# LiangZhaoPKUImperial/LinearSFM

Hardware: AMD Instinct MI355X
Metric: hierarchical linear map-joining solve wall-clock, NC3500-like stereo (all transforms + joins) (lower is better)
Workload: dtype f64

## Files before the change

include/lsfm.h:

```cpp
#ifndef LSFM_H
#define LSFM_H

#include <stddef.h>

#ifdef __cplusplus
extern "C" {
#endif

#define LSFM_OK 0
#define LSFM_ERR_ARG (-1)
#define LSFM_ERR_NO_DEVICE (-2)
#define LSFM_ERR_HIP (-3)
#define LSFM_ERR_OOM (-4)
#define LSFM_ERR_INTERNAL (-5)
#define LSFM_ERR_IO (-6)
#define LSFM_ERR_NOT_SPD (-7)
#define LSFM_NOT_CONVERGED 1

typedef struct lsfm_context lsfm_context;

typedef struct lsfm_map {
	int Ref, FRef, m, n, nU, nW;
	int ScaP, Fix, Sign, FScaP, FFix;
	int* stno;
// ... 75 lines not shown
int lsfm_gn_linearise_timed(lsfm_context* ctx, const lsfm_map* maps, int N, int type, const lsfm_map* x, const double* weight,
                            lsfm_map* out, double* obj, double* b, double* times, int* counts);
int lsfm_gn_linearise_features(lsfm_context* ctx, const lsfm_map* maps, int N, int type, const lsfm_map* x, const double* weight,
                               const double* fweight, lsfm_map* out, double* obj, double* b);
int lsfm_gn_linearise_features_timed(lsfm_context* ctx, const lsfm_map* maps, int N, int type, const lsfm_map* x, const double* weight,
                                     const double* fweight, lsfm_map* out, double* obj, double* b, double* times, int* counts);

int lsfm_map_covariance(lsfm_context* ctx, const lsfm_map* map, int mono, double* pose_cov, double* feat_cov, double* pair_cov, int cap_blocks, int* nnzb);
int lsfm_map_covariance_timed(lsfm_context* ctx, const lsfm_map* map, int mono, double* pose_cov, double* feat_cov, double* pair_cov, int cap_blocks, int* nnzb,
                              double* times);

int lsfm_map_covariance_columns(lsfm_context* ctx, const lsfm_map* map, int mono, const int* poses, int k, double* pose_cols, double* feat_cols,
                                double* joint, int* steps, double* last_corr);
int lsfm_map_covariance_columns_timed(lsfm_context* ctx, const lsfm_map* map, int mono, const int* poses, int k, double* pose_cols, double* feat_cols,
                                      double* joint, int* steps, double* last_corr, double* times);

int lsfm_map_covariance_feature_columns(lsfm_context* ctx, const lsfm_map* map, int mono, const int* feats, int k, double* pose_cols, double* feat_cols,
                                        double* joint, int* steps, double* last_corr);
int lsfm_map_feature_pair_gate(lsfm_context* ctx, const lsfm_map* map, int mono, const int* pairs, int K, double* d2, double* cov_diff, int* steps,
                               double* last_corr);
int lsfm_map_covariance_feature_columns_timed(lsfm_context* ctx, const lsfm_map* map, int mono, const int* feats, int k, double* pose_cols,
                                              double* feat_cols, double* joint, int* steps, double* last_corr, double* times);
int lsfm_map_feature_pair_gate_timed(lsfm_context* ctx, const lsfm_map* map, int mono, const int* pairs, int K, double* d2, double* cov_diff, int* steps,
                                     double* last_corr, double* times);

int lsfm_map_merge_features(lsfm_context* ctx, const lsfm_map* map, int mono, const int* pairs, int K, lsfm_map* out, double* d2, int* dof, int* rep,
                            int* steps, double* last_corr);
int lsfm_map_merge_features_timed(lsfm_context* ctx, const lsfm_map* map, int mono, const int* pairs, int K, lsfm_map* out, double* d2, int* dof,
                                  int* rep, int* steps, double* last_corr, double* times);
int lsfm_merge_structure(const lsfm_map* map, const int* pairs, int K, int* rep, int* photo, int* feature, int* FBlock, int* sptr, int* sidx, int cap_w,
                         int* info, char* why, int why_cap);

int lsfm_map_feature_pair_candidates(lsfm_context* ctx, const lsfm_map* map, const double* feat_cov, double radius, double tau, int* pairs, double* dist2,
                                     double* q, long long cap, long long* count);
int lsfm_map_feature_pair_candidates_timed(lsfm_context* ctx, const lsfm_map* map, const double* feat_cov, double radius, double tau, int* pairs,
                                           double* dist2, double* q, long long cap, long long* count, double* times, long long* info);

#define LSFM_JOINT_GATE_MAX 2048
int lsfm_map_feature_pair_joint_gate(lsfm_context* ctx, const lsfm_map* map, int mono, const int* pairs, int K, const int* order, double tau, int* status,
                                     double* delta, double* d2, double* joint_C, int* accepted, int* implied, double* D2, int* steps, double* last_corr);
int lsfm_map_feature_pair_joint_gate_timed(lsfm_context* ctx, const lsfm_map* map, int mono, const int* pairs, int K, const int* order, double tau,
                                           int* status, double* delta, double* d2, double* joint_C, int* accepted, int* implied, double* D2, int* steps,
                                           double* last_corr, double* times);
int lsfm_selftest_pair_select(lsfm_context* ctx, int K, const double* C, const double* d, const int* ends, const int* order, double tau, int* status,
                              double* delta, double* D2, int* accepted, int* implied);

int lsfm_map_marginalise(lsfm_context* ctx, const lsfm_map* map, const unsigned char* drop, lsfm_map* out);
int lsfm_map_marginalise_timed(lsfm_context* ctx, const lsfm_map* map, const unsigned char* drop, lsfm_map* out, double* times);

int lsfm_map_marginalise_poses(lsfm_context* ctx, const lsfm_map* map, int mono, const unsigned char* keep_pose, const unsigned char* drop_feat,
                               lsfm_map* out);
int lsfm_map_marginalise_poses_timed(lsfm_context* ctx, const lsfm_map* map, int mono, const unsigned char* keep_pose, const unsigned char* drop_feat,
                                     lsfm_map* out, double* times, int* info);
int lsfm_marg_pose_structure(const lsfm_map* map, int mono, const unsigned char* keep_pose, const unsigned char* drop_feat, unsigned char* drop,
                             int* comp, int* nptr, int* nidx, int cap_n, int* bd, int* Ui, int* Uj, int cap_u, int* info, char* why, int why_cap);

int lsfm_gn_structure(const lsfm_map* maps, int N, int type, const lsfm_map* x, int want_slots, int want_coalesce, int* info, int* map_hubs,
                      int* wdst, int* fptrJ, int* photoJ, int cap_wj, int* UiJ, int* UjJ, int cap_uj, int* photo, int* feature, int* FBlock,
                      int cap_w, int* Ui, int* Uj, int cap_u, int* slot_map, int* slot_a, int* slot_b, int* slot_count, int cap_s, char* why,
                      int why_cap);

int lsfm_inverse_v(lsfm_context* ctx, double* V, int m, int n);
int lsfm_solve_features(lsfm_context* ctx, const double* W, const double* IV, const double* ea, const double* eb, const double* dpa, double* dpb,
                        int m, int n, const int* mapCor, const int* photo);

int lsfm_schur_pattern(lsfm_context* ctx, const int* Ui, const int* Uj, const int* photo, const int* feature, int m, int n, int nU, int nW,
                       int* rowptr, int* colidx, int cap, int* nnzb);

int lsfm_symbolic_analyse(int m, const int* rowptr, const int* colidx, const int* origin, int reps, int* perm, int* colptr, int* rowidx,
                          int cap, int* info, double* avg_ms);

typedef struct lsfm_tree lsfm_tree;
int lsfm_tree_upload(lsfm_context* ctx, const lsfm_map* maps, int N, int mono, lsfm_tree** out);
int lsfm_tree_run(lsfm_context* ctx, lsfm_tree* tree, lsfm_stats* stats);
int lsfm_tree_set_final_reanchor(lsfm_tree* tree, int on);
int lsfm_tree_set_plans(lsfm_tree* tree, int on);
int lsfm_tree_download(lsfm_context* ctx, lsfm_tree* tree, lsfm_map* out);
int lsfm_tree_set_stop_level(lsfm_tree* tree, int levels);
int lsfm_tree_node_count(lsfm_context* ctx, lsfm_tree* tree);
int lsfm_tree_download_node(lsfm_context* ctx, lsfm_tree* tree, int k, lsfm_map* out);
int lsfm_tree_download_state(lsfm_context* ctx, lsfm_tree* tree, int* m, int* n, int* stno, double* stVal, size_t cap);
void lsfm_tree_free(lsfm_context* ctx, lsfm_tree* tree);
size_t lsfm_tree_export_size(lsfm_context* ctx, lsfm_tree* tree);
int lsfm_tree_export_dev(lsfm_context* ctx, lsfm_tree* tree, void* dst, size_t cap);
#define LSFM_PACK_HEADER_BYTES 256
size_t lsfm_packed_size(const void* host_header256);
int lsfm_tree_upload_dev(lsfm_context* ctx, const void* const* packed, int N, int mono, lsfm_tree** out);
int lsfm_tree_export_reduced_size(lsfm_context* ctx, lsfm_tree* tree, const int* keep_ids, int nkeep, size_t* bytes);
int lsfm_tree_export_reduced_dev(lsfm_context* ctx, lsfm_tree* tree, const int* keep_ids, int nkeep, void* dst, size_t cap);
int lsfm_tree_export_reduced_dev_timed(lsfm_context* ctx, lsfm_tree* tree, const int* keep_ids, int nkeep, void* dst, size_t cap, double* times);
int lsfm_tree_reload_dev(lsfm_context* ctx, lsfm_tree* tree, const void* const* packed, int N);

#define LSFM_DTYPE_F64 0
#define LSFM_DTYPE_I64 1
typedef int (*lsfm_allreduce_fn)(void* user, size_t offset_bytes, size_t count, int dtype, void* hip_stream);
int lsfm_tree_set_comm(lsfm_tree* tree, int rank, int world, lsfm_allreduce_fn fn, void* user, void* dev_buf, size_t dev_bytes);
int lsfm_tree_set_comm_blocks(lsfm_tree* tree, int block_maps);
int lsfm_tree_export_slice_sizes(lsfm_context* ctx, lsfm_tree* tree, int nslices, size_t* sizes);
int lsfm_tree_export_slice_dev(lsfm_context* ctx, lsfm_tree* tree, int nslices, int slice, void* dst, size_t cap);

int lsfm_divide_conquer(lsfm_context* ctx, const lsfm_map* maps, int N, int mono, lsfm_map* out, lsfm_stats* stats);

int lsfm_read_localmap(const char* path, int mono, lsfm_map* out);
int lsfm_read_localmaps(const char* dir, int first, int count, int mono, int threads, lsfm_map* out, int* failed);
int lsfm_write_localmap(const char* path, int mono, const lsfm_map* map);
int lsfm_write_mapset(const char* path, const lsfm_map* maps, int N, int mono);
int lsfm_mapset_info(const char* path, int* N, int* mono);
int lsfm_mapset_stamp(const char* path, unsigned long long* stamp, const unsigned long long* set_to);
int lsfm_read_mapset(const char* path, int mono, int first, int count, int threads, lsfm_map* out);
int lsfm_save_covariances(const char* pose_path, const char* feat_path, const int* stno, int m, int n, const double* pose_cov, const double* feat_cov);
int lsfm_read_covariances(const char* path, int k, int* ids, double* cov, int cap, int* count);
int lsfm_save_cov_columns(const char* path, const int* stno, int m, const int* poses, int k, const double* pose_cols);
int lsfm_read_cov_columns(const char* path, int* ids_q, int* ids_p, double* blocks, int cap, int* count);
int lsfm_save_pair_gate(const char* path, const int* ids, int K, const double* d2, const double* cov_diff);
int lsfm_read_pair_gate(const char* path, int* ids_f, int* ids_g, double* d2, double* cov_diff, int cap, int* count);
int lsfm_save_merge_report(const char* path, int K, int removed, int dof, double d2, const int* ids);
int lsfm_read_merge_report(const char* path, int* K, int* removed, int* dof, double* d2, int* ids, int cap);
int lsfm_save_joint_gate(const char* path, const int* ids, int K, const int* status, const double* d2, const double* delta, int accepted, int implied,
                         double D2);
int lsfm_read_joint_gate(const char* path, int* ids, int* status, double* d2, double* delta, int cap, int* head, double* D2);
int lsfm_save_pair_list(const char* path, const int* ids, long long K);
int lsfm_read_pair_list(const char* path, int* ids, long long cap, long long* count);
int lsfm_save_state(const char* path, const double* st, const int* stno, int n);
int lsfm_save_state_bin(const char* path, const double* st, const int* stno, int n);
int lsfm_save_poses(const char* pose_path, const char* feat_path, const int* stno, const double* st, int n);

int lsfm_spmv_bench(lsfm_context* ctx, int m, const int* rowptr, const int* colidx, const double* val,
                    const double* x, double* y, int reps, double* avg_ms, double* algorithmic_bytes);

int lsfm_wstream_bench(lsfm_context* ctx, long long nblocks, int mode, int reps, double* avg_ms);

int lsfm_selftest_prims(lsfm_context* ctx, int cases, unsigned seed);

int lsfm_selftest_vinv(lsfm_context* ctx, const double* V, const double* eb, int n, int skip, double* IV, double* LY);

#define LSFM_SELFTEST_CHOL_INFO 16
int lsfm_selftest_chol(lsfm_context* ctx, int m, const int* rowptr, const int* colidx, const double* val, const int* origin, const unsigned char* fixed,
                       const int* pose_seg, int nseg, const double* r, int nrhs, int mode, double* z, double* dot, int* perm, int* colptr, int* rowidx,
                       double* L, double* Dinv, double* dscale, int cap_blocks, int* info);

#define LSFM_SELFTEST_CC_SWEEPS_INFO 16
int lsfm_selftest_cc_sweeps(lsfm_context* ctx, int m, const int* rowptr, const int* colidx, const double* val, const int* origin,
                            const unsigned char* fixed, const double* B, int R, const double* X, double* x, double* fwd, int* perm, double* dscale,
                            double* y, int* info);

int lsfm_selftest_transform(lsfm_context* ctx, const lsfm_map* maps, int N, int mono, const int* tref, const int* tscap, const int* tfix,
                            int alias_passthrough, lsfm_map* out);

int lsfm_selftest_small(lsfm_context* ctx, int G, const int* pose_off, const int* feat_off, const int* u_off, const unsigned char* active,
                        const double* U, const int* Ui, const int* Uj, const double* W, const int* photo, const int* feature, int nW, const double* V,
                        const double* ea, const double* eb, const double* x0, const unsigned char* fixed, int strips, double* x_pose, double* x_feat,
                        int* status, double* max_rel);

#ifdef __cplusplus
}
#endif
#endif
```

linearsfm_amd/api.py:

```python
from __future__ import annotations

import ctypes as C
import os

import numpy as np

_HERE = os.path.dirname(os.path.abspath(__file__))
LIB_PATH = os.path.join(_HERE, "liblsfm_hip.so")
_LIB = None

LSFM_OK = 0
LSFM_NOT_CONVERGED = 1


class LsfmMap(C.Structure):
    _fields_ = [("Ref", C.c_int), ("FRef", C.c_int), ("m", C.c_int), ("n", C.c_int), ("nU", C.c_int), ("nW", C.c_int),
                ("ScaP", C.c_int), ("Fix", C.c_int), ("Sign", C.c_int), ("FScaP", C.c_int), ("FFix", C.c_int),
                ("stno", C.POINTER(C.c_int)), ("stVal", C.POINTER(C.c_double)),
                ("U", C.POINTER(C.c_double)), ("Ui", C.POINTER(C.c_int)), ("Uj", C.POINTER(C.c_int)),
                ("W", C.POINTER(C.c_double)), ("photo", C.POINTER(C.c_int)), ("feature", C.POINTER(C.c_int)),
                ("V", C.POINTER(C.c_double)), ("FBlock", C.POINTER(C.c_int)), ("pose_origin", C.POINTER(C.c_int))]


class LsfmStats(C.Structure):
    _fields_ = [("t_total_ms", C.c_double), ("t_transform_ms", C.c_double), ("t_join_ms", C.c_double),
                ("t_schur_ms", C.c_double), ("t_pcg_ms", C.c_double), ("t_backsub_ms", C.c_double),
                ("pcg_iterations", C.c_long), ("spmv_launches", C.c_long), ("spmv_ms", C.c_double),
                ("spmv_bytes", C.c_double), ("spmv_nnzb_upper_last", C.c_long), ("spmv_rows_last", C.c_long),
                ("max_rel_residual", C.c_double), ("levels", C.c_int), ("joins", C.c_int), ("transforms", C.c_int),
                ("not_converged", C.c_int), ("schur_launches", C.c_long), ("trf_launches", C.c_long),
                ("schur_ms", C.c_double), ("schur_bytes", C.c_double), ("trf_ms", C.c_double), ("trf_bytes", C.c_double),
                ("schur_flops", C.c_double), ("upload_ms", C.c_double), ("attempts", C.c_int),
                ("s_digest", C.c_ulonglong), ("factor_digest", C.c_ulonglong), ("dist_solves", C.c_int), ("dist_work_total", C.c_double), ("dist_work_shared", C.c_double), ("refactor_mismatch", C.c_int), ("s_rebuild_mismatch", C.c_int), ("small_levels", C.c_int), ("t_small_ms", C.c_double)]

    def as_dict(self):
        return {k: getattr(self, k) for k, _ in self._fields_}


class LsfmError(RuntimeError):
    pass


ALLREDUCE_FN = C.CFUNCTYPE(C.c_int, C.c_void_p, C.c_size_t, C.c_size_t, C.c_int, C.c_void_p)
LSFM_DTYPE_F64, LSFM_DTYPE_I64 = 0, 1
JOINT_GATE_MAX = 2048
JOINT_GATE_TAU = 11.344866730144373


def lib():
    global _LIB
    if _LIB is None:
        if not os.path.exists(LIB_PATH):
            raise LsfmError(f"{LIB_PATH} is missing: build it with `python -c 'import __graft_entry__ as g; g.build()'` "
                            "(hipcc --offload-arch=gfx950).  There is no CPU fallback.")
        L = C.CDLL(LIB_PATH)
        P = C.POINTER
        dp, ip, vp = P(C.c_double), P(C.c_int), C.c_void_p
        L.lsfm_context_create.argtypes = [C.c_int, C.c_size_t, P(vp)]
        L.lsfm_context_destroy.argtypes = [vp]
        L.lsfm_context_destroy.restype = None
        L.lsfm_set_pcg.argtypes = [vp, C.c_double, C.c_int]
        L.lsfm_set_precision.argtypes = [vp, C.c_int]
        L.lsfm_set_small_solve.argtypes = [vp, C.c_int]
        L.lsfm_set_spmv_variant.argtypes = [vp, C.c_int]
        L.lsfm_set_covcols_panel.argtypes = [vp, C.c_int]
        L.lsfm_last_error.argtypes = [vp]
        L.lsfm_last_error.restype = C.c_char_p
        L.lsfm_stream.argtypes = [vp]
        L.lsfm_stream.restype = vp
        L.lsfm_map_release.argtypes = [P(LsfmMap)]
        L.lsfm_map_release.restype = None
        L.lsfm_transform_stereo.argtypes = [vp, P(LsfmMap), C.c_int, P(LsfmMap)]
        L.lsfm_transform_mono.argtypes = [vp, P(LsfmMap), C.c_int, C.c_int, C.c_int, P(LsfmMap)]
        L.lsfm_join_stereo.argtypes = [vp, P(LsfmMap), P(LsfmMap), P(LsfmMap), dp, dp]
        L.lsfm_join_mono.argtypes = [vp, P(LsfmMap), P(LsfmMap), P(LsfmMap), dp, dp]
        L.lsfm_solve_stereo.argtypes = [vp, dp, dp, dp, dp, dp, dp, ip, ip, ip, ip, C.c_int, C.c_int, C.c_int, C.c_int, dp]
        L.lsfm_solve_mono.argtypes = [vp, dp, dp, dp, dp, dp, dp, ip, ip, ip, ip, C.c_int, C.c_int, C.c_int, C.c_int,
                                      C.c_int, C.c_int, C.c_int, C.c_int, C.c_int, dp]
        L.lsfm_tree_upload.argtypes = [vp, P(LsfmMap), C.c_int, C.c_int, P(vp)]
        L.lsfm_tree_run.argtypes = [vp, vp, P(LsfmStats)]
        L.lsfm_tree_set_final_reanchor.argtypes = [vp, C.c_int]
        L.lsfm_tree_set_plans.argtypes = [vp, C.c_int]
        L.lsfm_tree_export_size.argtypes = [vp, vp]
        L.lsfm_tree_export_size.restype = C.c_size_t
        L.lsfm_tree_export_dev.argtypes = [vp, vp, vp, C.c_size_t]
        L.lsfm_packed_size.argtypes = [vp]
        L.lsfm_packed_size.restype = C.c_size_t
        L.lsfm_tree_upload_dev.argtypes = [vp, P(vp), C.c_int, C.c_int, P(vp)]
        L.lsfm_tree_reload_dev.argtypes = [vp, vp, P(vp), C.c_int]
        L.lsfm_tree_set_comm.argtypes = [vp, C.c_int, C.c_int, ALLREDUCE_FN, vp, vp, C.c_size_t]
        L.lsfm_tree_set_comm_blocks.argtypes = [vp, C.c_int]
        L.lsfm_tree_export_slice_sizes.argtypes = [vp, vp, C.c_int, P(C.c_size_t)]
        L.lsfm_tree_export_slice_dev.argtypes = [vp, vp, C.c_int, C.c_int, vp, C.c_size_t]
        L.lsfm_tree_download.argtypes = [vp, vp, P(LsfmMap)]
        L.lsfm_tree_set_stop_level.argtypes = [vp, C.c_int]
        L.lsfm_tree_node_count.argtypes = [vp, vp]
        L.lsfm_tree_download_node.argtypes = [vp, vp, C.c_int, P(LsfmMap)]
        L.lsfm_tree_download_state.argtypes = [vp, vp, ip, ip, ip, dp, C.c_size_t]
        L.lsfm_tree_free.argtypes = [vp, vp]
        L.lsfm_tree_free.restype = None
        L.lsfm_divide_conquer.argtypes = [vp, P(LsfmMap), C.c_int, C.c_int, P(LsfmMap), P(LsfmStats)]
        L.lsfm_read_localmap.argtypes = [C.c_char_p, C.c_int, P(LsfmMap)]
        L.lsfm_write_localmap.argtypes = [C.c_char_p, C.c_int, P(LsfmMap)]
        L.lsfm_read_localmaps.argtypes = [C.c_char_p, C.c_int, C.c_int, C.c_int, C.c_int, P(LsfmMap), P(C.c_int)]
        L.lsfm_write_mapset.argtypes = [C.c_char_p, P(LsfmMap), C.c_int, C.c_int]
        L.lsfm_mapset_info.argtypes = [C.c_char_p, P(C.c_int), P(C.c_int)]
        L.lsfm_read_mapset.argtypes = [C.c_char_p, C.c_int, C.c_int, C.c_int, C.c_int, P(LsfmMap)]
        L.lsfm_save_state_bin.argtypes = [C.c_char_p, P(C.c_double), P(C.c_int), C.c_int]
        L.lsfm_save_state.argtypes = [C.c_char_p, dp, ip, C.c_int]
        L.lsfm_save_poses.argtypes = [C.c_char_p, C.c_char_p, ip, dp, C.c_int]
        L.lsfm_schur_pattern.argtypes = [vp, ip, ip, ip, ip, C.c_int, C.c_int, C.c_int, C.c_int, ip, ip, C.c_int, ip]
        L.lsfm_symbolic_analyse.argtypes = [C.c_int, ip, ip, ip, C.c_int, ip, ip, ip, C.c_int, ip, dp]
        L.lsfm_inverse_v.argtypes = [vp, dp, C.c_int, C.c_int]
        L.lsfm_selftest_vinv.argtypes = [vp, dp, dp, C.c_int, C.c_int, dp, dp]
        L.lsfm_gn_polish.argtypes = [vp, P(LsfmMap), C.c_int, C.c_int, P(LsfmMap), C.c_int, dp, dp, ip]
        L.lsfm_gn_polish_robust.argtypes = [vp, P(LsfmMap), C.c_int, C.c_int, P(LsfmMap), C.c_int, C.c_int, C.c_double, dp, dp, ip, dp, dp]
        L.lsfm_map_chi2.argtypes = [vp, P(LsfmMap), C.c_int, C.c_int, P(LsfmMap), dp, ip]
        L.lsfm_map_feature_chi2.argtypes = [vp, P(LsfmMap), C.c_int, C.c_int, P(LsfmMap), dp, dp]
        L.lsfm_gn_polish_robust_features.argtypes = [vp, P(LsfmMap), C.c_int, C.c_int, P(LsfmMap), C.c_int, C.c_int, C.c_double, dp, dp, ip, dp, dp]
        L.lsfm_gn_linearise.argtypes = [vp, P(LsfmMap), C.c_int, C.c_int, P(LsfmMap), dp, P(LsfmMap), dp, dp]
        L.lsfm_gn_linearise_timed.argtypes = [vp, P(LsfmMap), C.c_int, C.c_int, P(LsfmMap), dp, P(LsfmMap), dp, dp, dp, ip]
        L.lsfm_gn_linearise_features.argtypes = [vp, P(LsfmMap), C.c_int, C.c_int, P(LsfmMap), dp, dp, P(LsfmMap), dp, dp]
        L.lsfm_gn_linearise_features_timed.argtypes = [vp, P(LsfmMap), C.c_int, C.c_int, P(LsfmMap), dp, dp, P(LsfmMap), dp, dp, dp, ip]
        L.lsfm_solve_features.argtypes = [vp, dp, dp, dp, dp, dp, dp, C.c_int, C.c_int, ip, ip]
        L.lsfm_map_covariance.argtypes = [vp, P(LsfmMap), C.c_int, dp, dp, dp, C.c_int, ip]
        L.lsfm_map_covariance_timed.argtypes = [vp, P(LsfmMap), C.c_int, dp, dp, dp, C.c_int, ip, dp]
        L.lsfm_save_covariances.argtypes = [C.c_char_p, C.c_char_p, ip, C.c_int, C.c_int, dp, dp]
        L.lsfm_read_covariances.argtypes = [C.c_char_p, C.c_int, ip, dp, C.c_int, ip]
        L.lsfm_map_covariance_columns.argtypes = [vp, P(LsfmMap), C.c_int, ip, C.c_int, dp, dp, dp, ip, dp]
        L.lsfm_map_covariance_columns_timed.argtypes = [vp, P(LsfmMap), C.c_int, ip, C.c_int, dp, dp, dp, ip, dp, dp]
        L.lsfm_map_covariance_feature_columns.argtypes = [vp, P(LsfmMap), C.c_int, ip, C.c_int, dp, dp, dp, ip, dp]
        L.lsfm_map_covariance_feature_columns_timed.argtypes = [vp, P(LsfmMap), C.c_int, ip, C.c_int, dp, dp, dp, ip, dp, dp]
        L.lsfm_map_feature_pair_gate.argtypes = [vp, P(LsfmMap), C.c_int, ip, C.c_int, dp, dp, ip, dp]
        L.lsfm_map_feature_pair_gate_timed.argtypes = [vp, P(LsfmMap), C.c_int, ip, C.c_int, dp, dp, ip, dp, dp]
        L.lsfm_map_merge_features.argtypes = [vp, P(LsfmMap), C.c_int, ip, C.c_int, P(LsfmMap), dp, ip, ip, ip, dp]
        L.lsfm_map_merge_features_timed.argtypes = [vp, P(LsfmMap), C.c_int, ip, C.c_int, P(LsfmMap), dp, ip, ip, ip, dp, dp]
        L.lsfm_map_feature_pair_joint_gate.argtypes = [vp, P(LsfmMap), C.c_int, ip, C.c_int, ip, C.c_double, ip, dp, dp, dp, ip, ip, dp, ip, dp]
        L.lsfm_map_feature_pair_joint_gate_timed.argtypes = [vp, P(LsfmMap), C.c_int, ip, C.c_int, ip, C.c_double, ip, dp, dp, dp, ip, ip, dp, ip, dp, dp]
        L.lsfm_selftest_pair_select.argtypes = [vp, C.c_int, dp, dp, ip, ip, C.c_double, ip, dp, dp, ip, ip]
        L.lsfm_save_joint_gate.argtypes = [C.c_char_p, ip, C.c_int, ip, dp, dp, C.c_int, C.c_int, C.c_double]
        L.lsfm_read_joint_gate.argtypes = [C.c_char_p, ip, ip, dp, dp, C.c_int, ip, dp]
        L.lsfm_merge_structure.argtypes = [P(LsfmMap), ip, C.c_int, ip, ip, ip, ip, ip, ip, C.c_int, ip, C.c_char_p, C.c_int]
        llp = P(C.c_longlong)
        L.lsfm_map_feature_pair_candidates.argtypes = [vp, P(LsfmMap), dp, C.c_double, C.c_double, ip, dp, dp, C.c_longlong, llp]
        L.lsfm_map_feature_pair_candidates_timed.argtypes = [vp, P(LsfmMap), dp, C.c_double, C.c_double, ip, dp, dp, C.c_longlong, llp, dp, llp]
        L.lsfm_save_pair_list.argtypes = [C.c_char_p, ip, C.c_longlong]
        L.lsfm_read_pair_list.argtypes = [C.c_char_p, ip, C.c_longlong, llp]
        L.lsfm_save_merge_report.argtypes = [C.c_char_p, C.c_int, C.c_int, C.c_int, C.c_double, ip]
        L.lsfm_read_merge_report.argtypes = [C.c_char_p, ip, ip, ip, dp, ip, C.c_int]
        L.lsfm_save_cov_columns.argtypes = [C.c_char_p, ip, C.c_int, ip, C.c_int, dp]
        L.lsfm_read_cov_columns.argtypes = [C.c_char_p, ip, ip, dp, C.c_int, ip]
        L.lsfm_save_pair_gate.argtypes = [C.c_char_p, ip, C.c_int, dp, dp]
        L.lsfm_read_pair_gate.argtypes = [C.c_char_p, ip, ip, dp, dp, C.c_int, ip]
        L.lsfm_map_marginalise.argtypes = [vp, P(LsfmMap), P(C.c_ubyte), P(LsfmMap)]
        L.lsfm_map_marginalise_timed.argtypes = [vp, P(LsfmMap), P(C.c_ubyte), P(LsfmMap), dp]
        ub = P(C.c_ubyte)
        L.lsfm_map_marginalise_poses.argtypes = [vp, P(LsfmMap), C.c_int, ub, ub, P(LsfmMap)]
        L.lsfm_map_marginalise_poses_timed.argtypes = [vp, P(LsfmMap), C.c_int, ub, ub, P(LsfmMap), dp, ip]
        L.lsfm_marg_pose_structure.argtypes = [P(LsfmMap), C.c_int, ub, ub, ub, ip, ip, ip, C.c_int, ip, ip, ip, C.c_int, ip, C.c_char_p, C.c_int]
        L.lsfm_gn_structure.argtypes = [P(LsfmMap), C.c_int, C.c_int, P(LsfmMap), C.c_int, C.c_int, ip, ip, ip, ip, ip, C.c_int, ip, ip, C.c_int, ip, ip, ip,
                                        C.c_int, ip, ip, C.c_int, ip, ip, ip, ip, C.c_int, C.c_char_p, C.c_int]
        L.lsfm_tree_export_reduced_size.argtypes = [vp, vp, ip, C.c_int, P(C.c_size_t)]
        L.lsfm_tree_export_reduced_dev.argtypes = [vp, vp, ip, C.c_int, vp, C.c_size_t]
        L.lsfm_tree_export_reduced_dev_timed.argtypes = [vp, vp, ip, C.c_int, vp, C.c_size_t, dp]
        L.lsfm_spmv_bench.argtypes = [vp, C.c_int, ip, ip, dp, dp, dp, C.c_int, dp, dp]
        L.lsfm_wstream_bench.argtypes = [vp, C.c_longlong, C.c_int, C.c_int, dp]
        L.lsfm_selftest_prims.argtypes = [vp, C.c_int, C.c_uint]
        L.lsfm_selftest_chol.argtypes = [vp, C.c_int, ip, ip, dp, ip, P(C.c_ubyte), ip, C.c_int, dp, C.c_int, C.c_int, dp, dp, ip, ip, ip, dp, dp, dp,
                                         C.c_int, ip]
        L.lsfm_selftest_cc_sweeps.argtypes = [vp, C.c_int, ip, ip, dp, ip, P(C.c_ubyte), dp, C.c_int, dp, dp, dp, ip, dp, dp, ip]
        L.lsfm_selftest_transform.argtypes = [vp, P(LsfmMap), C.c_int, C.c_int, ip, ip, ip, C.c_int, P(LsfmMap)]
        L.lsfm_selftest_small.argtypes = [vp, C.c_int, ip, ip, ip, ub, dp, ip, ip, dp, ip, ip, C.c_int, dp, dp, dp, dp, ub, C.c_int, dp, dp, ip, dp]
        _LIB = L
    return _LIB


EXPORTS = ["lsfm_context_create", "lsfm_context_destroy", "lsfm_set_pcg", "lsfm_set_precision", "lsfm_set_small_solve", "lsfm_set_spmv_variant", "lsfm_set_covcols_panel", "lsfm_last_error", "lsfm_stream",
           "lsfm_map_release", "lsfm_transform_stereo", "lsfm_transform_mono", "lsfm_join_stereo", "lsfm_join_mono",
           "lsfm_solve_stereo", "lsfm_solve_mono", "lsfm_tree_upload", "lsfm_tree_run", "lsfm_tree_set_final_reanchor",
           "lsfm_tree_download", "lsfm_tree_set_stop_level", "lsfm_tree_node_count", "lsfm_tree_download_node", "lsfm_tree_download_state", "lsfm_tree_set_plans", "lsfm_tree_export_size", "lsfm_tree_export_dev", "lsfm_packed_size",
           "lsfm_tree_upload_dev", "lsfm_tree_reload_dev", "lsfm_tree_set_comm", "lsfm_tree_set_comm_blocks", "lsfm_tree_export_slice_sizes", "lsfm_tree_export_slice_dev",
           "lsfm_tree_free", "lsfm_divide_conquer", "lsfm_read_localmap", "lsfm_read_localmaps", "lsfm_write_localmap", "lsfm_write_mapset", "lsfm_mapset_info", "lsfm_mapset_stamp", "lsfm_read_mapset", "lsfm_save_state_bin", "lsfm_save_state", "lsfm_save_poses", "lsfm_gn_polish",
           "lsfm_gn_polish_robust", "lsfm_map_chi2", "lsfm_map_feature_chi2", "lsfm_gn_polish_robust_features", "lsfm_gn_linearise", "lsfm_gn_linearise_timed",
           "lsfm_gn_linearise_features", "lsfm_gn_linearise_features_timed",
           "lsfm_spmv_bench", "lsfm_wstream_bench", "lsfm_selftest_prims", "lsfm_selftest_chol", "lsfm_selftest_cc_sweeps", "lsfm_selftest_transform", "lsfm_selftest_small", "lsfm_schur_pattern", "lsfm_symbolic_analyse", "lsfm_inverse_v", "lsfm_selftest_vinv", "lsfm_solve_features",
           "lsfm_map_covariance", "lsfm_map_covariance_timed",
           "lsfm_save_covariances", "lsfm_read_covariances",
           "lsfm_map_covariance_columns", "lsfm_map_covariance_columns_timed", "lsfm_save_cov_columns", "lsfm_read_cov_columns",
           "lsfm_map_covariance_feature_columns", "lsfm_map_covariance_feature_columns_timed", "lsfm_map_feature_pair_gate", "lsfm_map_feature_pair_gate_timed", "lsfm_save_pair_gate", "lsfm_read_pair_gate",
           "lsfm_map_merge_features", "lsfm_map_merge_features_timed", "lsfm_merge_structure", "lsfm_save_merge_report", "lsfm_read_merge_report",
           "lsfm_map_feature_pair_candidates", "lsfm_map_feature_pair_candidates_timed", "lsfm_save_pair_list", "lsfm_read_pair_list",
           "lsfm_map_feature_pair_joint_gate", "lsfm_map_feature_pair_joint_gate_timed", "lsfm_selftest_pair_select", "lsfm_save_joint_gate", "lsfm_read_joint_gate",
           "lsfm_map_marginalise", "lsfm_map_marginalise_timed", "lsfm_tree_export_reduced_size", "lsfm_tree_export_reduced_dev",
           "lsfm_tree_export_reduced_dev_timed", "lsfm_map_marginalise_poses", "lsfm_map_marginalise_poses_timed", "lsfm_marg_pose_structure", "lsfm_gn_structure"]


def _c(a, dtype):
    return np.ascontiguousarray(a, dtype=dtype).reshape(-1)


def _ptr(a, ctype):
    return a.ctypes.data_as(C.POINTER(ctype))


class HostMap:

    def __init__(self, d):
        g = d if isinstance(d, dict) else d.__dict__
        self.stno = _c(g["stno"], np.int32); self.stVal = _c(g["stVal"], np.float64)
        self.U = _c(g["U"], np.float64); self.Ui = _c(g["Ui"], np.int32); self.Uj = _c(g["Uj"], np.int32)
        self.W = _c(g["W"], np.float64); self.photo = _c(g["photo"], np.int32); self.feature = _c(g["feature"], np.int32)
        self.V = _c(g["V"], np.float64); self.FBlock = _c(g["FBlock"], np.int32)
        c = LsfmMap()
        c.Ref = int(g["Ref"]); c.FRef = int(g.get("FRef", g["Ref"])); c.m = int(g["m"]); c.n = int(g["n"])
        c.nU = len(self.Ui); c.nW = len(self.photo)
        c.ScaP = int(g.get("ScaP", 0)); c.Fix = int(g.get("Fix", 0)); c.Sign = int(g.get("Sign", 1))
        c.FScaP = int(g.get("FScaP", c.ScaP)); c.FFix = int(g.get("FFix", c.Fix))
        c.stno = _ptr(self.stno, C.c_int); c.stVal = _ptr(self.stVal, C.c_double)
        c.U = _ptr(self.U, C.c_double); c.Ui = _ptr(self.Ui, C.c_int); c.Uj = _ptr(self.Uj, C.c_int)
        c.W = _ptr(self.W, C.c_double); c.photo = _ptr(self.photo, C.c_int); c.feature = _ptr(self.feature, C.c_int)
        c.V = _ptr(self.V, C.c_double); c.FBlock = _ptr(self.FBlock, C.c_int)
        if g.get("pose_origin") is not None:
            self.pose_origin = _c(g["pose_origin"], np.int32)
            c.pose_origin = _ptr(self.pose_origin, C.c_int)
        self.c = c


def _arr(ptr, n, dtype):
    if n == 0:
        return np.zeros(0, dtype)
    return np.ctypeslib.as_array(ptr, shape=(n,)).astype(dtype, copy=True)


def map_to_dict(g: LsfmMap, release=True):
    r = 6 * g.m + 3 * g.n
    d = dict(Ref=g.Ref, FRef=g.FRef, m=g.m, n=g.n, nU=g.nU, nW=g.nW, ScaP=g.ScaP, Fix=g.Fix, Sign=g.Sign,
             FScaP=g.FScaP, FFix=g.FFix,
             stno=_arr(g.stno, r, np.int32), stVal=_arr(g.stVal, r, np.float64),
             U=_arr(g.U, 36 * g.nU, np.float64).reshape(-1, 36), Ui=_arr(g.Ui, g.nU, np.int32), Uj=_arr(g.Uj, g.nU, np.int32),
             W=_arr(g.W, 18 * g.nW, np.float64).reshape(-1, 18), photo=_arr(g.photo, g.nW, np.int32),
             feature=_arr(g.feature, g.nW, np.int32), V=_arr(g.V, 9 * g.n, np.float64).reshape(-1, 9),
             FBlock=_arr(g.FBlock, g.n, np.int32))
    if g.pose_origin:
        d["pose_origin"] = _arr(g.pose_origin, g.m, np.int32)
    if release:
        lib().lsfm_map_release(C.byref(g))
    return d


def _gn_args(maps, G):
    hms = [HostMap(d) for d in maps]
    arr = (LsfmMap * len(hms))(*[h.c for h in hms])
    x = LsfmMap()
    stno = _c(G["stno"], np.int32)
    st = np.array(np.asarray(G["stVal"], np.float64), copy=True)
    x.m, x.n, x.Ref, x.FRef = int(G["m"]), int(G["n"]), int(G["Ref"]), int(G.get("FRef", G["Ref"]))
    x.ScaP, x.Fix, x.Sign = int(G.get("ScaP", 0)), int(G.get("Fix", 0)), int(G.get("Sign", 1))
    x.FScaP, x.FFix = int(G.get("FScaP", x.ScaP)), int(G.get("FFix", x.Fix))
    x.stno, x.stVal = _ptr(stno, C.c_int), _ptr(st, C.c_double)
    org = None
    if G.get("pose_origin") is not None:
        org = _c(G["pose_origin"], np.int32)
        x.pose_origin = _ptr(org, C.c_int)
    return hms, arr, x, (stno, st, org)


class Context:

    def __init__(self, device=0, arena_bytes=0):
        self._h = C.c_void_p()
        rc = lib().lsfm_context_create(int(device), int(arena_bytes), C.byref(self._h))
        if rc != 0:
            self._h = None
            raise LsfmError(f"lsfm_context_create failed (rc={rc}): no usable HIP device -- there is no CPU fallback")

    def close(self):
        if self._h:
            lib().lsfm_context_destroy(self._h)
            self._h = None

    def __del__(self):
        try:
            self.close()
        except Exception:
            pass

    def _check(self, rc, what):
        if rc < 0:
            raise LsfmError(f"{what} failed (rc={rc}): {lib().lsfm_last_error(self._h).decode()}")
        return rc

    def set_pcg(self, rel_tol=1e-12, max_steps=0):
        self._check(lib().lsfm_set_pcg(self._h, float(rel_tol), int(max_steps)), "lsfm_set_pcg")

    def set_precision(self, mixed):
        self._check(lib().lsfm_set_precision(self._h, 1 if mixed else 0), "lsfm_set_precision")

    def set_small_solve(self, max_poses=5):
        self._check(lib().lsfm_set_small_solve(self._h, int(max_poses)), "lsfm_set_small_solve")

    def set_spmv_variant(self, variant):
        self._check(lib().lsfm_set_spmv_variant(self._h, int(variant)), "lsfm_set_spmv_variant")

    def set_covcols_panel(self, variant):
        self._check(lib().lsfm_set_covcols_panel(self._h, int(variant)), "lsfm_set_covcols_panel")

    def stream(self):
        return lib().lsfm_stream(self._h)

    def tree_reload_dev(self, tree, dev_ptrs):
        arr = (C.c_void_p * len(dev_ptrs))(*[C.c_void_p(int(p)) for p in dev_ptrs])
        self._check(lib().lsfm_tree_reload_dev(self._h, tree, arr, len(dev_ptrs)), "lsfm_tree_reload_dev")

    def transform(self, d, mono, Ref, ScaP=0, Fix=0):
        hm = HostMap(d)
        out = LsfmMap()
        if mono:
            rc = lib().lsfm_transform_mono(self._h, C.byref(hm.c), int(Ref), int(ScaP), int(Fix), C.byref(out))
        else:
            rc = lib().lsfm_transform_stereo(self._h, C.byref(hm.c), int(Ref), C.byref(out))
        self._check(rc, "lsfm_transform")
        return map_to_dict(out)

    def join(self, dEnd, dCur, mono):
        he, hc = HostMap(dEnd), HostMap(dCur)
        out = LsfmMap()
        m = he.c.m + hc.c.m - (2 if mono else 0)
        eP = np.zeros(6 * m)
        eF = np.zeros(3 * (he.c.n + hc.c.n))
        fn = lib().lsfm_join_mono if mono else lib().lsfm_join_stereo
        rc = self._check(fn(self._h, C.byref(he.c), C.byref(hc.c), C.byref(out), _ptr(eP, C.c_double), _ptr(eF, C.c_double)),
                         "lsfm_join")
        j = map_to_dict(out)
        return j, eP, eF[:3 * j["n"]], rc

    def solve(self, j, eP, eF, mono, sa=None, x0=None):
        m, n = int(j["m"]), int(j["n"])
        st = np.zeros(6 * m + 3 * n)
# ... 443 lines not shown
        h = HostMap(d)
        fl = np.ascontiguousarray(np.asarray(drop).astype(bool), dtype=np.uint8).reshape(-1)
        if len(fl) != h.c.n:
            raise LsfmError(f"marginalise: {len(fl)} flags for {h.c.n} features")
        out = LsfmMap()
        t = np.zeros(3)
        self._check(lib().lsfm_map_marginalise_timed(self._h, C.byref(h.c), _ptr(fl, C.c_ubyte), C.byref(out), _ptr(t, C.c_double) if times else None),
                    "lsfm_map_marginalise")
        g = map_to_dict(out)
        if times:
            return g, dict(zip(("structure_ms", "values_ms", "emit_ms"), t.tolist()))
        return g

    def marginalise_poses(self, d, mono, keep_pose, drop_feat=None, times=False, info=False):
        h = HostMap(d)
        kp = np.ascontiguousarray(np.asarray(keep_pose).astype(bool), dtype=np.uint8).reshape(-1)
        if len(kp) != h.c.m:
            raise LsfmError(f"marginalise_poses: {len(kp)} flags for {h.c.m} poses")
        fl = None
        if drop_feat is not None:
            fl = np.ascontiguousarray(np.asarray(drop_feat).astype(bool), dtype=np.uint8).reshape(-1)
            if len(fl) != h.c.n:
                raise LsfmError(f"marginalise_poses: {len(fl)} flags for {h.c.n} features")
        out = LsfmMap()
        t = np.zeros(5)
        inf = np.zeros(8, np.int32)
        rc = self._check(lib().lsfm_map_marginalise_poses_timed(self._h, C.byref(h.c), int(mono), _ptr(kp, C.c_ubyte), _ptr(fl, C.c_ubyte) if fl is not None else None,
                                                                C.byref(out), _ptr(t, C.c_double), _ptr(inf, C.c_int)), "lsfm_map_marginalise_poses")
        if rc != 0:
            raise LsfmError(f"lsfm_map_marginalise_poses: {rc} pivot(s) floored -- the dropped poses' own system is too close to singular")
        res = [map_to_dict(out)]
        if times:
            res.append(dict(zip(("stage_a_ms", "structure_ms", "factor_ms", "sweeps_ms", "syrk_emit_ms"), t.tolist())))
        if info:
            res.append(dict(zip(MARG_POSES_INFO, (int(v) for v in inf))))
        return res[0] if len(res) == 1 else tuple(res)

    def spmv_bench(self, rowptr, colidx, val, x, reps=20):
        rowptr = _c(rowptr, np.int32); colidx = _c(colidx, np.int32); val = _c(val, np.float64); x = _c(x, np.float64)
        m = len(rowptr) - 1
        y = np.zeros(6 * m)
        ms, by = C.c_double(), C.c_double()
        self._check(lib().lsfm_spmv_bench(self._h, m, _ptr(rowptr, C.c_int), _ptr(colidx, C.c_int), _ptr(val, C.c_double),
                                          _ptr(x, C.c_double), _ptr(y, C.c_double), int(reps), C.byref(ms), C.byref(by)),
                    "lsfm_spmv_bench")
        return y, ms.value, by.value


def _wstream(self, nblocks, mode, reps=10):
    ms = C.c_double()
    self._check(lib().lsfm_wstream_bench(self._h, int(nblocks), int(mode), int(reps), C.byref(ms)), "lsfm_wstream_bench")
    return ms.value


Context.wstream_bench = _wstream


def _selftest_prims(self, cases=64, seed=1):
    self._check(lib().lsfm_selftest_prims(self._h, int(cases), int(seed)), "lsfm_selftest_prims")


Context.selftest_prims = _selftest_prims

SELFTEST_CHOL_INFO = ("blocks", "leaf_tasks", "leaf_columns", "task0_outer", "groups", "group_levels", "fused_levels", "split_levels", "max_rows_below",
                      "d_err", "floored")


def _selftest_chol(self, rowptr, colidx, val, r, origin=None, fixed=None, pose_seg=None, nseg=1, mode=0):
    rowptr = _c(rowptr, np.int32); colidx = _c(colidx, np.int32); val = _c(val, np.float64)
    m = len(rowptr) - 1
    if m < 1 or len(colidx) != rowptr[-1] or len(val) != 36 * len(colidx):
        raise LsfmError("selftest_chol: rowptr / colidx / val do not fit together")
    r = np.ascontiguousarray(r, dtype=np.float64).reshape(-1, 6 * m)
    nrhs = r.shape[0]
    org = _c(origin, np.int32) if origin is not None else None
    fx = np.ascontiguousarray(np.asarray(fixed).astype(bool), dtype=np.uint8).reshape(-1) if fixed is not None else None
    seg = _c(pose_seg, np.int32) if pose_seg is not None else np.zeros(m, np.int32)
    if (org is not None and len(org) != m) or (fx is not None and len(fx) != 6 * m) or len(seg) != m:
        raise LsfmError("selftest_chol: origin / fixed / pose_seg do not fit m")
    cap = int(symbolic_analyse(rowptr, colidx, org)["info"][0])
    z = np.zeros((nrhs, 6 * m)); dot = np.zeros((nrhs, int(nseg)))
    perm = np.zeros(m, np.int32); colptr = np.zeros(m + 1, np.int32); rowidx = np.zeros(cap, np.int32)
    Lb = np.zeros((cap, 6, 6)); Dinv = np.zeros((m, 6, 6)); dscale = np.zeros(6 * m)
    info = np.zeros(16, np.int32)
    rc = lib().lsfm_selftest_chol(self._h, m, _ptr(rowptr, C.c_int), _ptr(colidx, C.c_int), _ptr(val, C.c_double),
                                  _ptr(org, C.c_int) if org is not None else None, _ptr(fx, C.c_ubyte) if fx is not None else None,
                                  _ptr(seg, C.c_int), int(nseg), _ptr(r, C.c_double), nrhs, int(mode), _ptr(z, C.c_double), _ptr(dot, C.c_double),
                                  _ptr(perm, C.c_int), _ptr(colptr, C.c_int), _ptr(rowidx, C.c_int), _ptr(Lb, C.c_double), _ptr(Dinv, C.c_double),
                                  _ptr(dscale, C.c_double), cap, _ptr(info, C.c_int))
    self._check(rc, "lsfm_selftest_chol")
    return dict(z=z, dot=dot, perm=perm, colptr=colptr, rowidx=rowidx, L=Lb, Dinv=Dinv, dscale=dscale,
                info=dict(zip(SELFTEST_CHOL_INFO, (int(v) for v in info))))


Context.selftest_chol = _selftest_chol

SELFTEST_CC_SWEEPS_INFO = ("leaf_tasks", "groups", "group_levels", "max_rows_below", "width_mask", "fwd_task_launches", "fwd_group_launches",
                           "fwd_panel_launches", "bwd_panel_launches", "panel", "d_err", "floored")


def _selftest_cc_sweeps(self, rowptr, colidx, val, B, origin=None, fixed=None, X=None):
    rowptr = _c(rowptr, np.int32); colidx = _c(colidx, np.int32); val = _c(val, np.float64)
    m = len(rowptr) - 1
    if m < 1 or len(colidx) != rowptr[-1] or len(val) != 36 * len(colidx):
        raise LsfmError("selftest_cc_sweeps: rowptr / colidx / val do not fit together")
    B = np.ascontiguousarray(B, dtype=np.float64)
    if B.ndim != 2 or B.shape[0] != 6 * m:
        raise LsfmError("selftest_cc_sweeps: B is not [6 m, R]")
    R = B.shape[1]
    org = _c(origin, np.int32) if origin is not None else None
    fx = np.ascontiguousarray(np.asarray(fixed).astype(bool), dtype=np.uint8).reshape(-1) if fixed is not None else None
    if (org is not None and len(org) != m) or (fx is not None and len(fx) != 6 * m):
        raise LsfmError("selftest_cc_sweeps: origin / fixed do not fit m")
    Xc = y = None
    if X is not None:
        Xc = np.ascontiguousarray(X, dtype=np.float64)
        if Xc.shape != B.shape:
            raise LsfmError("selftest_cc_sweeps: X is not shaped like B")
        y = np.zeros_like(B)
    x = np.zeros_like(B); fwd = np.zeros_like(B)
    perm = np.zeros(m, np.int32); dscale = np.zeros(6 * m)
    info = np.zeros(16, np.int32)
    rc = lib().lsfm_selftest_cc_sweeps(self._h, m, _ptr(rowptr, C.c_int), _ptr(colidx, C.c_int), _ptr(val, C.c_double),
                                       _ptr(org, C.c_int) if org is not None else None, _ptr(fx, C.c_ubyte) if fx is not None else None,
                                       _ptr(B, C.c_double), R, _ptr(Xc, C.c_double) if Xc is not None else None, _ptr(x, C.c_double),
                                       _ptr(fwd, C.c_double), _ptr(perm, C.c_int), _ptr(dscale, C.c_double),
                                       _ptr(y, C.c_double) if y is not None else None, _ptr(info, C.c_int))
    self._check(rc, "lsfm_selftest_cc_sweeps")
    return dict(x=x, fwd=fwd, perm=perm, dscale=dscale, y=y, info=dict(zip(SELFTEST_CC_SWEEPS_INFO, (int(v) for v in info))))


Context.selftest_cc_sweeps = _selftest_cc_sweeps


def _selftest_transform(self, dicts, mono, targets, alias=False):
    hms = [HostMap(d) for d in dicts]
    N = len(hms)
    if N < 1 or len(targets) != N:
        raise LsfmError("selftest_transform: one target per map")
    t = np.zeros((3, N), np.int32)
    for b, tg in enumerate(targets):
        t[:, b] = (-1, 0, 0) if tg is None else (tuple(tg) + (0, 0))[:3] if isinstance(tg, (tuple, list)) else (int(tg), 0, 0)
    arr = (LsfmMap * N)(*[h.c for h in hms])
    out = (LsfmMap * N)()
    rc = lib().lsfm_selftest_transform(self._h, arr, N, int(bool(mono)), _ptr(t[0], C.c_int), _ptr(t[1], C.c_int), _ptr(t[2], C.c_int),
                                       int(bool(alias)), out)
    self._check(rc, "lsfm_selftest_transform")
    return [map_to_dict(out[b]) for b in range(N)]


Context.selftest_transform = _selftest_transform


def _selftest_small(self, B, strips=0, active=None, fixed=None, x0=None, prefill=None):
    po, fo, uo = (_c(B[k], np.int32) for k in ("pose_off", "feat_off", "u_off"))
    G = len(po) - 1
    if G < 1 or len(fo) != G + 1 or len(uo) != G + 1:
        raise LsfmError("selftest_small: pose_off / feat_off / u_off must have one entry per system and one more")
    M, NF, NU = int(po[-1]), int(fo[-1]), int(uo[-1])
    U = _c(B["U"], np.float64); Ui = _c(B["Ui"], np.int32); Uj = _c(B["Uj"], np.int32)
    W = _c(B["W"], np.float64); ph = _c(B["photo"], np.int32); fe = _c(B["feature"], np.int32); V = _c(B["V"], np.float64)
    ea = _c(B["ea"], np.float64); eb = _c(B["eb"], np.float64)
    nW = len(ph)
    if (len(U), len(Ui), len(Uj)) != (36 * NU, NU, NU) or (len(W), len(fe)) != (18 * nW, nW) or (len(V), len(ea), len(eb)) != (9 * NF, 6 * M, 3 * NF):
        raise LsfmError("selftest_small: the arrays do not fit the offsets")
    flags = lambda a, n, what: None if a is None else _fit(np.ascontiguousarray(np.asarray(a).astype(bool), dtype=np.uint8).reshape(-1), n, what)
    act, fx = flags(active, G, "active"), flags(fixed, 6 * M, "fixed")
    x0 = None if x0 is None else _fit(_c(x0, np.float64), 6 * M, "x0")
    if prefill is None:
        xp, xf = np.full(6 * M, np.nan), np.full(3 * NF, np.nan)
    else:
        xp, xf = _fit(np.array(_c(prefill[0], np.float64)), 6 * M, "prefill"), _fit(np.array(_c(prefill[1], np.float64)), 3 * NF, "prefill")
    st = np.zeros(2, np.int32)
    mr = C.c_double()
    d, i, opt = C.c_double, C.c_int, lambda a, t: None if a is None else _ptr(a, t)
    rc = lib().lsfm_selftest_small(self._h, G, _ptr(po, i), _ptr(fo, i), _ptr(uo, i), opt(act, C.c_ubyte), _ptr(U, d), _ptr(Ui, i), _ptr(Uj, i),
                                   _ptr(W, d), _ptr(ph, i), _ptr(fe, i), nW, _ptr(V, d), _ptr(ea, d), _ptr(eb, d), opt(x0, d), opt(fx, C.c_ubyte),
                                   int(strips), _ptr(xp, d), _ptr(xf, d), _ptr(st, i), C.byref(mr))
    self._check(rc, "lsfm_selftest_small")
    return xp, xf, st, mr.value


def _fit(a, n, what):
    if len(a) != n:
        raise LsfmError(f"selftest_small: {what} has {len(a)} entries, not {n}")
    return a


Context.selftest_small = _selftest_small


def symbolic_analyse(rowptr, colidx, origin=None, reps=1):
    rowptr = _c(rowptr, np.int32); colidx = _c(colidx, np.int32)
    m = len(rowptr) - 1
    org = _c(origin, np.int32) if origin is not None else None
    info = np.zeros(8, np.int32)
    perm = np.zeros(m, np.int32); colptr = np.zeros(m + 1, np.int32)
    ms = C.c_double()
    lib().lsfm_symbolic_analyse(m, _ptr(rowptr, C.c_int), _ptr(colidx, C.c_int), _ptr(org, C.c_int) if org is not None else None, 1,
                                _ptr(perm, C.c_int), _ptr(colptr, C.c_int), None, 0, _ptr(info, C.c_int), None)
    rowidx = np.zeros(max(int(info[0]), 1), np.int32)
    rc = lib().lsfm_symbolic_analyse(m, _ptr(rowptr, C.c_int), _ptr(colidx, C.c_int), _ptr(org, C.c_int) if org is not None else None, int(reps),
                                     _ptr(perm, C.c_int), _ptr(colptr, C.c_int), _ptr(rowidx, C.c_int), len(rowidx), _ptr(info, C.c_int), C.byref(ms))
    if rc:
        raise LsfmError(f"lsfm_symbolic_analyse failed (rc={rc}): malformed pattern")
    return dict(perm=perm, colptr=colptr, rowidx=rowidx[:int(info[0])], info=info, ms=ms.value)


MARG_POSES_INFO = ("dropped", "boundary", "components", "blocks", "chunks", "leaf_tasks", "groups", "group_levels")


def marg_pose_structure(d, mono, keep_pose, drop_feat=None):
    h = HostMap(d)
    m, n = h.c.m, h.c.n
    kp = None if keep_pose is None else np.ascontiguousarray(np.asarray(keep_pose).astype(bool), dtype=np.uint8).reshape(-1)
    fl = None if drop_feat is None else np.ascontiguousarray(np.asarray(drop_feat).astype(bool), dtype=np.uint8).reshape(-1)
    if (kp is not None and len(kp) != m) or (fl is not None and len(fl) != n):
        raise LsfmError("marg_pose_structure: the flags do not fit the map")
    info = np.zeros(8, np.int32)
    why = C.create_string_buffer(512)
    ub = C.c_ubyte
    args = (C.byref(h.c), int(mono), _ptr(kp, ub) if kp is not None else None, _ptr(fl, ub) if fl is not None else None)
    rc = lib().lsfm_marg_pose_structure(*args, None, None, None, None, 0, None, None, None, 0, _ptr(info, C.c_int), why, len(why))
    if rc:
        raise LsfmError(f"lsfm_marg_pose_structure failed (rc={rc}): {why.value.decode()}")
    drop = np.zeros(max(n, 1), np.uint8); comp = np.zeros(m, np.int32); nptr = np.zeros(m + 1, np.int32); bd = np.zeros(m, np.int32)
    nidx = np.zeros(max(int(info[4]), 1), np.int32); Ui = np.zeros(max(int(info[3]), 1), np.int32); Uj = np.zeros_like(Ui)
    rc = lib().lsfm_marg_pose_structure(*args, _ptr(drop, ub), _ptr(comp, C.c_int), _ptr(nptr, C.c_int), _ptr(nidx, C.c_int), len(nidx), _ptr(bd, C.c_int),
                                        _ptr(Ui, C.c_int), _ptr(Uj, C.c_int), len(Ui), _ptr(info, C.c_int), why, len(why))
    if rc:
        raise LsfmError(f"lsfm_marg_pose_structure failed (rc={rc}): {why.value.decode()}")
    nc = int(info[2])
    return dict(drop=drop[:n].astype(bool), comp=comp, nptr=nptr[:nc + 1].copy(), nidx=nidx[:int(info[4])].copy(), bd=bd[:int(info[1])].copy(),
                Ui=Ui[:int(info[3])].copy(), Uj=Uj[:int(info[3])].copy(), info=info)


MERGE_STRUCTURE_INFO = ("n", "nW", "classes", "removed", "summed_blocks")


def merge_structure(d, pairs):
    h = HostMap(d)
    pr = _c(pairs, np.int32)
    K = len(pr) // 2
    info = np.zeros(8, np.int32)
    why = C.create_string_buffer(512)
    p = lambda a: _ptr(a, C.c_int)
    head = (C.byref(h.c), p(pr) if K else None, K)
    rc = lib().lsfm_merge_structure(*head, None, None, None, None, None, None, 0, p(info), why, len(why))
    if rc:
        raise LsfmError(f"lsfm_merge_structure failed (rc={rc}): {why.value.decode()}")
    v = dict(zip(MERGE_STRUCTURE_INFO, (int(i) for i in info)))
    n, nW = h.c.n, h.c.nW
    cap = max(nW, 1)
    rep, photo, feature, FBlock = np.zeros(max(n, 1), np.int32), np.zeros(cap, np.int32), np.zeros(cap, np.int32), np.zeros(max(n, 1), np.int32)
    sptr, sidx = np.zeros(cap + 1, np.int32), np.zeros(cap, np.int32)
    rc = lib().lsfm_merge_structure(*head, p(rep), p(photo), p(feature), p(FBlock), p(sptr), p(sidx), cap, p(info), why, len(why))
    if rc:
        raise LsfmError(f"lsfm_merge_structure failed (rc={rc}): {why.value.decode()}")
    return dict(rep=rep[:n], photo=photo[:v["nW"]], feature=feature[:v["nW"]], FBlock=FBlock[:v["n"]], sptr=sptr[:v["nW"] + 1], sidx=sidx[:nW], info=v)


GN_STRUCTURE_INFO = ("M", "NFG", "P", "FI", "NUJ", "NWJ", "nU", "nW", "slots", "contributors")


def gn_structure(maps, mono, G, slots=False, coalesce=False):
    hms, arr, x, keep = _gn_args(maps, G)
    N = len(hms)
    info = np.zeros(10, np.int32)
    why = C.create_string_buffer(512)
    head = (arr, N, 1 if mono else 0, C.byref(x), int(bool(slots)), int(bool(coalesce)), _ptr(info, C.c_int))
    rc = lib().lsfm_gn_structure(*head, None, None, None, None, 0, None, None, 0, None, None, None, 0, None, None, 0, None, None, None, None, 0, why, len(why))
    if rc:
        raise LsfmError(f"lsfm_gn_structure failed (rc={rc}): {why.value.decode()}")
    v = dict(zip(GN_STRUCTURE_INFO, (int(i) for i in info)))
    z = lambda n: np.zeros(max(n, 1), np.int32)
    hubs, wdst, fptrJ, photoJ, UiJ, UjJ = z(3 * N), z(v["FI"]), z(v["NFG"] + 1), z(v["NWJ"]), z(v["NUJ"]), z(v["NUJ"])
    photo, feature, FBlock, Ui, Uj = z(v["nW"]), z(v["nW"]), z(v["NFG"]), z(v["nU"]), z(v["nU"])
    sm, sa, sb, sc = z(v["slots"]), z(v["slots"]), z(v["slots"]), z(v["slots"])
    p = lambda a: _ptr(a, C.c_int)
    rc = lib().lsfm_gn_structure(*head, p(hubs), p(wdst), p(fptrJ), p(photoJ), len(photoJ), p(UiJ), p(UjJ), len(UiJ), p(photo), p(feature), p(FBlock),
                                 len(photo), p(Ui), p(Uj), len(Ui), p(sm), p(sa), p(sb), p(sc), len(sm), why, len(why))
    if rc:
        raise LsfmError(f"lsfm_gn_structure failed (rc={rc}): {why.value.decode()}")
    return dict(info=v, map_hubs=hubs.reshape(N, 3), wdst=wdst[:v["FI"]], fptrJ=fptrJ, photoJ=photoJ[:v["NWJ"]], UiJ=UiJ[:v["NUJ"]], UjJ=UjJ[:v["NUJ"]],
                photo=photo[:v["nW"]], feature=feature[:v["nW"]], FBlock=FBlock[:v["NFG"] if coalesce else 0], Ui=Ui[:v["nU"]], Uj=Uj[:v["nU"]],
                slot_map=sm[:v["slots"]], slot_a=sa[:v["slots"]], slot_b=sb[:v["slots"]], slot_count=sc[:v["slots"]])


LSFM_NODE_MAGIC = 1279870541


def read_localmap(path, mono):
    g = LsfmMap()
    rc = lib().lsfm_read_localmap(str(path).encode(), int(mono), C.byref(g))
    if rc:
        raise LsfmError(f"lsfm_read_localmap({path}) failed (rc={rc})")
    return map_to_dict(g)


def write_localmap(path, d, mono):
    hm = HostMap(d)
    rc = lib().lsfm_write_localmap(str(path).encode(), int(mono), C.byref(hm.c))
    if rc:
        raise LsfmError(f"lsfm_write_localmap({path}) failed (rc={rc})")


def write_mapset(path, maps, mono):
    hms = [HostMap(d) for d in maps]
    arr = (LsfmMap * len(hms))(*[h.c for h in hms])
    rc = lib().lsfm_write_mapset(str(path).encode(), arr, len(hms), int(mono))
    if rc:
        raise LsfmError(f"lsfm_write_mapset({path}) failed (rc={rc})")


def mapset_info(path):
    n, mono = C.c_int(0), C.c_int(0)
    if lib().lsfm_mapset_info(str(path).encode(), C.byref(n), C.byref(mono)):
        return None
    return n.value, bool(mono.value)


def read_mapset(path, mono, first=0, count=None, threads=0):
    info = mapset_info(path)
    if info is None:
        raise LsfmError(f"{path}: not a map-set cache")
    if count is None:
        count = info[0] - first
    arr = (LsfmMap * max(count, 1))()
    rc = lib().lsfm_read_mapset(str(path).encode(), int(mono), int(first), int(count), int(threads), arr)
    if rc:
        raise LsfmError(f"lsfm_read_mapset({path}) failed (rc={rc})")
    return [map_to_dict(arr[k]) for k in range(count)]


def read_localmaps(directory, count, mono, first=1, threads=0):
    arr = (LsfmMap * count)()
    bad = C.c_int(0)
    rc = lib().lsfm_read_localmaps(str(directory).encode(), int(first), int(count), int(mono), int(threads), arr, C.byref(bad))
    if rc:
        raise LsfmError(f"lsfm_read_localmaps({directory}) failed at localmap_{bad.value}.txt (rc={rc})")
    return [map_to_dict(arr[k]) for k in range(count)]

# ... 146 lines not shown
```

linearsfm_amd/csrc/lsfm_capi.hip:

```cpp
#include <climits>
#include <cmath>
#include <cstring>

#include "lsfm_internal.hpp"
#include "lsfm_marg.hpp"
#include "lsfm_solve.hpp"
#include "lsfm_system.hpp"
#include "lsfm_tree.hpp"

using namespace lsfm;

namespace {

template <class F> int guarded(lsfm_context* ctx, F&& f)
{
	if (!ctx) return LSFM_ERR_ARG;
	struct Reset {
		lsfm_context* c;
		~Reset() { c->timed.clear(); c->ev_next = 0; c->plan = nullptr; }
	} reset{ ctx };
	try
	{
		if (hipSetDevice(ctx->device) != hipSuccess) return LSFM_ERR_NO_DEVICE;
		return f();
// ... 638 lines not shown
	return lsfm_map_merge_features_timed(ctx, map, mono, pairs, K, out, d2, dof, rep, steps, last_corr, nullptr);
}

int lsfm_map_feature_pair_candidates_timed(lsfm_context* ctx, const lsfm_map* map, const double* feat_cov, double radius, double tau, int* pairs,
                                           double* dist2, double* q, long long cap, long long* count, double* times, long long* info)
{
	if (!map || map->m < 0 || map->n < 0 || (map->n && !map->stVal) || !count) return LSFM_ERR_ARG;
	long long cnt = 0;
	const int rc = guarded(ctx, [&]() { return map_feature_pair_candidates(ctx, map, feat_cov, radius, tau, pairs, dist2, q, cap, &cnt, times, info); });
	*count = cnt;
	return rc;
}

int lsfm_map_feature_pair_candidates(lsfm_context* ctx, const lsfm_map* map, const double* feat_cov, double radius, double tau, int* pairs, double* dist2,
                                     double* q, long long cap, long long* count)
{
	return lsfm_map_feature_pair_candidates_timed(ctx, map, feat_cov, radius, tau, pairs, dist2, q, cap, count, nullptr, nullptr);
}

int lsfm_inverse_v(lsfm_context* ctx, double* V, int m, int n)
{
	(void)m;
	if (n < 0 || (n && !V)) return LSFM_ERR_ARG;
	return guarded(ctx, [&]() { return inverse_v(ctx, V, n); });
}

int lsfm_selftest_vinv(lsfm_context* ctx, const double* V, const double* eb, int n, int skip, double* IV, double* LY)
{
	if (n < 0 || skip < 0 || skip > 1 || (n && (!V || !eb || !IV || !LY))) return LSFM_ERR_ARG;
	return guarded(ctx, [&]() { return vinv_selftest(ctx, V, eb, n, skip, IV, LY); });
}

int lsfm_solve_features(lsfm_context* ctx, const double* W, const double* IV, const double* ea, const double* eb, const double* dpa, double* dpb,
                        int m, int n, const int* mapCor, const int* photo)
{
	(void)ea;
	if (m <= 0 || n < 0 || !dpa || (n && (!W || !IV || !eb || !dpb || !mapCor || !photo))) return LSFM_ERR_ARG;
	return guarded(ctx, [&]() { return solve_features(ctx, W, IV, eb, dpa, dpb, m, n, mapCor, photo); });
}

int lsfm_schur_pattern(lsfm_context* ctx, const int* Ui, const int* Uj, const int* photo, const int* feature, int m, int n, int nU, int nW, int* rowptr,
                       int* colidx, int cap, int* nnzb)
{
	if (m <= 0 || n < 0 || nU < 0 || nW < 0 || !rowptr || !colidx || !nnzb || (nU && (!Ui || !Uj)) || (nW && (!photo || !feature))) return LSFM_ERR_ARG;
	return guarded(ctx, [&]() {
		HostSystem h;
		h.m = m; h.n = n; h.nU = nU; h.nW = nW;
		h.Ui = Ui; h.Uj = Uj; h.photo = photo; h.feature = feature;
		SolveIO io;
		system_upload(ctx, h, 0, system_fptr(h, true), nullptr, io);
		int cnt = 0;
		const int* d_rowptr = nullptr;
		const int* d_colidx = nullptr;
		schur_pattern_only(ctx, io, &cnt, &d_rowptr, &d_colidx);
		*nnzb = cnt;
		if (cnt > cap) LSFM_FAIL(LSFM_ERR_ARG, "colidx too small for the pattern (" + std::to_string(cnt) + " blocks)");
		d2h(ctx, rowptr, d_rowptr, (size_t)(m + 1) * sizeof(int));
		d2h(ctx, colidx, d_colidx, (size_t)cnt * sizeof(int));
		return LSFM_OK;
	});
}

int lsfm_spmv_bench(lsfm_context* ctx, int m, const int* rowptr, const int* colidx, const double* val, const double* x, double* y,
                    int reps, double* avg_ms, double* algorithmic_bytes)
{
	if (!rowptr || !colidx || !val || !x || !y || m <= 0) return LSFM_ERR_ARG;
	return guarded(ctx, [&]() {
		ctx->ensure_arenas(((size_t)rowptr[m] * 480 + (size_t)m * 1000) * 2 + ((size_t)64 << 20));
		ctx->scratch.reset();
		return spmv_external(ctx, m, rowptr, colidx, val, x, y, reps, avg_ms, algorithmic_bytes);
	});
}

static bool block_csr_ok(int m, const int* rowptr, const int* colidx, const double* val)
{
	if (m <= 0 || !rowptr || !colidx || !val || rowptr[0] != 0) return false;
	for (int p = 0; p < m; p++)
	{
		if (rowptr[p + 1] <= rowptr[p] || colidx[rowptr[p]] != p) return false;
		for (int k = rowptr[p] + 1; k < rowptr[p + 1]; k++)
			if (colidx[k] <= colidx[k - 1] || colidx[k] >= m) return false;
	}
	return true;
}

int lsfm_selftest_chol(lsfm_context* ctx, int m, const int* rowptr, const int* colidx, const double* val, const int* origin, const unsigned char* fixed,
                       const int* pose_seg, int nseg, const double* r, int nrhs, int mode, double* z, double* dot, int* perm, int* colptr, int* rowidx,
                       double* L, double* Dinv, double* dscale, int cap_blocks, int* info)
{
	if (!block_csr_ok(m, rowptr, colidx, val) || !pose_seg || nseg <= 0 || !r || nrhs <= 0 || mode < 0 || mode > 3 || !z || !dot || !info || cap_blocks < 0)
		return LSFM_ERR_ARG;
	for (int p = 0; p < m; p++)
		if (pose_seg[p] < 0 || pose_seg[p] >= nseg) return LSFM_ERR_ARG;
	for (int i = 0; i < LSFM_SELFTEST_CHOL_INFO; i++) info[i] = 0;
	return guarded(ctx, [&]() {
		return chol_selftest(ctx, m, rowptr, colidx, val, origin, fixed, pose_seg, nseg, r, nrhs, mode, z, dot, perm, colptr, rowidx, L, Dinv, dscale, cap_blocks, info);
	});
}

int lsfm_selftest_cc_sweeps(lsfm_context* ctx, int m, const int* rowptr, const int* colidx, const double* val, const int* origin,
                            const unsigned char* fixed, const double* B, int R, const double* X, double* x, double* fwd, int* perm, double* dscale,
                            double* y, int* info)
{
	if (!block_csr_ok(m, rowptr, colidx, val) || !B || R < 1 || R > 192  || (X != nullptr) != (y != nullptr) || !info) return LSFM_ERR_ARG;
	for (int i = 0; i < LSFM_SELFTEST_CC_SWEEPS_INFO; i++) info[i] = 0;
	return guarded(ctx, [&]() { return cc_sweeps_selftest(ctx, m, rowptr, colidx, val, origin, fixed, B, R, X, x, fwd, perm, dscale, y, info); });
}

int lsfm_selftest_transform(lsfm_context* ctx, const lsfm_map* maps, int N, int mono, const int* tref, const int* tscap, const int* tfix,
                            int alias_passthrough, lsfm_map* out)
{
	if (!maps || N <= 0 || !tref || !out || (mono && (!tscap || !tfix))) return LSFM_ERR_ARG;
	for (int b = 0; b < N; b++) memset(&out[b], 0, sizeof out[b]);
	int rc = guarded(ctx, [&]() {
		ctx->ensure_arenas(estimate_arena(maps, N, 1));
		ctx->arena[0].reset(); ctx->arena[1].reset(); ctx->scratch.reset();
		DevBatch X, Y;
		batch_upload(ctx, ctx->arena[0], maps, N, mono != 0, X);
		std::vector<int> r(tref, tref + N), s(N, 0), f(N, 0);
		if (mono) { s.assign(tscap, tscap + N); f.assign(tfix, tfix + N); }
		transform_batch(ctx, ctx->arena[1], X, r, s, f, mono != 0, Y, alias_passthrough != 0);
		std::vector<int> delta(N, INT_MIN);
		if (Y.W_alias) d2h(ctx, delta.data(), Y.d_alias, (size_t)N * sizeof(int));
		for (int b = 0; b < N; b++)
		{
			batch_download_map(ctx, Y, b, mono != 0, &out[b]);
			if (delta[b] == INT_MIN || !out[b].nW) continue;
			d2h(ctx, out[b].W, Y.W_alias + ((ptrdiff_t)Y.w_off[b] + delta[b]) * 18, (size_t)out[b].nW * 18 * sizeof(double));
		}
		return LSFM_OK;
	});
	if (rc < 0) for (int b = 0; b < N; b++) lsfm_map_release(&out[b]);
	return rc;
}

int lsfm_selftest_small(lsfm_context* ctx, int G, const int* pose_off, const int* feat_off, const int* u_off, const unsigned char* active,
                        const double* U, const int* Ui, const int* Uj, const double* W, const int* photo, const int* feature, int nW, const double* V,
                        const double* ea, const double* eb, const double* x0, const unsigned char* fixed, int strips, double* x_pose, double* x_feat,
                        int* status, double* max_rel)
{
	if (G <= 0 || !pose_off || !feat_off || !u_off || !ea || !x_pose || !status || !max_rel || strips < 0 || nW < 0) return LSFM_ERR_ARG;
	const int M = pose_off[G], NF = feat_off[G], NU = u_off[G];
	if (M <= 0 || NF < 0 || NU < 0 || (NU && (!U || !Ui || !Uj)) || (nW && (!W || !photo || !feature)) || (NF && (!V || !eb || !x_feat))) return LSFM_ERR_ARG;
	status[0] = status[1] = 0; *max_rel = 0.0;
	return guarded(ctx, [&]() {
		HostSystem h;
		h.m = M; h.n = NF; h.nU = NU; h.nW = nW;
		h.Ui = Ui; h.Uj = Uj; h.photo = photo; h.feature = feature;
		h.U = U; h.W = W; h.V = V; h.ea = ea; h.eb = eb; h.x0 = x0;
		return small_selftest(ctx, G, pose_off, feat_off, u_off, active, h, fixed, strips, x_pose, x_feat, status, max_rel);
	});
}

int lsfm_wstream_bench(lsfm_context* ctx, long long nblocks, int mode, int reps, double* avg_ms)
{
	if (nblocks <= 0 || mode < 0 || mode > 2 || reps <= 0 || !avg_ms) return LSFM_ERR_ARG;
	return guarded(ctx, [&]() {
		ctx->ensure_arenas((size_t)nblocks * 144 * 2 + ((size_t)64 << 20));
		ctx->scratch.reset();
		return wstream_bench(ctx, nblocks, mode, reps, avg_ms);
	});
}
int lsfm_selftest_prims(lsfm_context* ctx, int cases, unsigned seed)
{
	if (cases <= 0) return LSFM_ERR_ARG;
	return guarded(ctx, [&]() { return prims_selftest(ctx, cases, seed); });
}

}
```

linearsfm_amd/csrc/lsfm_internal.hpp:

```cpp
#pragma once
#include <hip/hip_runtime.h>

#include <cstdint>
#include <cstdio>
#include <condition_variable>
#include <cstring>
#include <exception>
#include <functional>
#include <memory>
#include <mutex>
#include <thread>
#include <string>
#include <vector>

#include "../../include/lsfm.h"
#include "lsfm_map.hpp"

namespace lsfm {

struct Error { int code; std::string msg; };
struct DevBatch;
struct IndexHold;
struct SolvePlan;
struct PreLevel;
// ... 217 lines not shown
	hipEvent_t ev_half[2] = { nullptr, nullptr };
	unsigned long long generation = 0;
	hipStream_t stream2 = nullptr;
	hipEvent_t ord[lsfm::ORD_COUNT] = {};
	void quiesce_side_streams();
	std::shared_ptr<lsfm::EarlyPattern> early;
	hipStream_t stream3 = nullptr;
	lsfm::Arena sarena[2];
	std::shared_ptr<lsfm::PreLevel> pre;
	lsfm::LevelPlan pre_plan;
	int pre_plan_level = -1;
	std::unique_ptr<lsfm::HostWorker> worker;
	void drop_prepared() { pre.reset(); pre_plan = lsfm::LevelPlan(); pre_plan_level = -1; }
	double dbg_gap_ms = 0.0;
	std::vector<std::pair<const char*, double>> timeline;
	bool timeline_on = false;
	void mark(const char* what);
	bool in_tree_run = false;
	lsfm_stats* stats = nullptr;
	lsfm::LevelPlan* plan = nullptr;
	bool warm() const { return plan && plan->valid; }
	lsfm::RunStatsDev* d_run = nullptr;
	lsfm::Comm* comm = nullptr;
	std::vector<hipEvent_t> ev_pool;
	size_t ev_next = 0;
	struct Timed { hipEvent_t a, b; double* sink; };
	std::vector<Timed> timed;
	hipEvent_t pool_event();
	void defer_time(hipEvent_t a, hipEvent_t b, double* sink) { timed.push_back(Timed{ a, b, sink }); }
	void flush_times();
	void ensure_arenas(size_t bytes_each, bool start_small = false);
	bool grow_arenas();
	bool arena_small = false;
	size_t arena_bound = 0;
};

namespace lsfm {

struct OnStream {
	lsfm_context* c; hipStream_t& s; Arena* a;
	OnStream(lsfm_context* ctx, hipStream_t& other, Arena* arena = nullptr) : c(ctx), s(other), a(arena) { std::swap(c->stream, s); if (a) std::swap(c->scratch, *a); }
	~OnStream() { if (a) std::swap(c->scratch, *a); std::swap(c->stream, s); }
	OnStream(const OnStream&) = delete;
	OnStream& operator=(const OnStream&) = delete;
};
inline void wait_for(lsfm_context* ctx, hipStream_t s, Ord e) { LSFM_CHECK_HIP(hipStreamWaitEvent(s, ctx->ord[e], 0)); }
struct Fork {
	lsfm_context* c; hipStream_t main; OnStream on;
	Fork(lsfm_context* ctx, hipStream_t& side, Arena* arena = nullptr) : c(ctx), main(ctx->stream), on(ctx, side, arena) {}
	Fork(lsfm_context* ctx, hipStream_t& side, Ord start, bool record = true, Arena* arena = nullptr) : Fork(ctx, side, arena)
	{
		if (record) LSFM_CHECK_HIP(hipEventRecord(c->ord[start], main));
		wait_for(c, c->stream, start);
	}
	void done(Ord e) { LSFM_CHECK_HIP(hipEventRecord(c->ord[e], c->stream)); }
	void join(Ord e) { done(e); wait_for(c, main, e); }
};

void dev_exclusive_scan(lsfm_context* ctx, const int* in, int* out, size_t n);
void dev_sort_pairs_u64(lsfm_context* ctx, unsigned long long* keys, int* vals, size_t n, int end_bit, int begin_bit = 0);
void dev_sort_keys_u64(lsfm_context* ctx, const unsigned long long* keys, unsigned long long* sorted, size_t n, int begin_bit, int end_bit);
int d2h_int(lsfm_context* ctx, const int* dptr);
void d2h_ints(lsfm_context* ctx, const int* dptr, int* h, size_t n);
void h2d(lsfm_context* ctx, void* d, const void* h, size_t bytes);
struct HostPiece { const void* p; size_t bytes; };
void h2d_gather(lsfm_context* ctx, void* d, const std::vector<HostPiece>& pieces);
struct CopyBatch {
	lsfm_context* ctx;
	struct Item { void* dst; const void* src; size_t bytes; bool host; };
	std::vector<Item> items;
	explicit CopyBatch(lsfm_context* c) : ctx(c) {}
	void h2d(void* d, const void* h, size_t bytes) { if (bytes) items.push_back(Item{ d, h, bytes, true }); }
	void d2d(void* d, const void* s, size_t bytes) { if (bytes) items.push_back(Item{ d, s, bytes, false }); }
	void flush();
};
void d2h(lsfm_context* ctx, void* h, const void* d, size_t bytes);
void dev_zero(lsfm_context* ctx, void* d, size_t bytes);
void fill_async(hipStream_t s, void* d, int byte, size_t bytes);

void batch_upload(lsfm_context* ctx, Arena& ar, const lsfm_map* maps, int N, bool mono, DevBatch& out);
void batch_download_map(lsfm_context* ctx, const DevBatch& b, int k, bool mono, lsfm_map* out);
inline void map_new(lsfm_map& g, const lsfm_map* like, int m, int n, int nU, int nW, bool pose_origin)
{
	if (map_alloc(g, like, m, n, nU, nW, pose_origin) != LSFM_OK) throw Error{ LSFM_ERR_OOM, "out of host memory for the merged map" };
}
struct CopyBatch;
void batch_set_offsets(lsfm_context* ctx, Arena& ar, DevBatch& b, CopyBatch* cb = nullptr);
void batch_fill_maps(lsfm_context* ctx, DevBatch& b);
struct PackHeader {
	int magic, version, mono, m, n, nU, nW, Ref, FRef, ScaP, Fix, Sign, FScaP, FFix, pad0, pad1;
	unsigned long long total;
	unsigned long long off[12];
	unsigned long long pad[11];
};
static_assert(sizeof(PackHeader) == 256, "the header is the first 256 bytes of a pack");
#define LSFM_PACK_MAGIC 0x4d46534c
size_t pack_layout(PackHeader& h);
void batch_pack_map(lsfm_context* ctx, const DevBatch& b, int k, bool mono, void* dst, size_t cap);
void batch_slice_counts(lsfm_context* ctx, const DevBatch& b, int nslices, std::vector<int>& nf, std::vector<int>& nw);
void batch_pack_slice(lsfm_context* ctx, const DevBatch& b, bool mono, int nslices, int slice, int nf, int nw, void* dst, size_t cap);
void batch_unpack_maps(lsfm_context* ctx, Arena& ar, const void* const* packed, const PackHeader* hdr, int N, bool mono, DevBatch& out);
unsigned long long batch_structure_digest(lsfm_context* ctx, const DevBatch& b);

inline bool map_in_frame(const DevBatch& X, int b, int tref, int tscap, bool mono) { return X.Ref[b] == tref && (!mono || X.ScaP[b] == tscap); }
int level_targets(const DevBatch& X, bool mono, std::vector<int>& tref, std::vector<int>& tscap, std::vector<int>& tfix);
struct TrRedirect {
	const int* wbase = nullptr;
	const int* newf = nullptr;
	double* W = nullptr;
	int *photo = nullptr, *feature = nullptr, *srcf = nullptr;
};
using TrHook = std::function<TrRedirect(DevBatch& mid, const int* hub)>;
void transform_batch(lsfm_context* ctx, Arena& ar, const DevBatch& in, const std::vector<int>& target_ref,
                     const std::vector<int>& target_scap, const std::vector<int>& target_fix, bool mono, DevBatch& out,
                     bool alias_passthrough = false, const TrHook* hook = nullptr);

struct JoinWork;
struct SolveIO {
	int M = 0, NF = 0, NU = 0, NW = 0, nseg = 0;
	const int* d_pose_seg = nullptr;
	const int* d_feat_seg = nullptr;
	const unsigned char* d_seg_active = nullptr;
	const double* U = nullptr; const int *Ui = nullptr, *Uj = nullptr;
	const double* W = nullptr; const int *photo = nullptr, *fptr = nullptr;
	const double* V = nullptr;
	const double* ea = nullptr;
	const double* eb = nullptr;
	const double* x0 = nullptr;
	const unsigned char* d_fixed = nullptr;
	const int* d_pose_origin = nullptr;
	double* x_pose = nullptr;
	double* x_feat = nullptr;
	std::vector<int> seg_rows;
	const int *d_pose_off = nullptr, *d_feat_off = nullptr, *d_u_off = nullptr;
	const struct RhsFused* rhs = nullptr;
	const struct PatternSeed* seed = nullptr;
	bool index_arrays_at_evA = false;
	int step_hint = 0;
	bool caller_syncs = false;
};
struct SolveOutcome {
	int not_converged = 0;
	int steps_used = 0;
	const unsigned long long* keys = nullptr;
	int nnzb = 0;
	hipEvent_t end = nullptr;
};
int small_level_strips(const lsfm_context* ctx, int most_rows);
inline int most_rows(const std::vector<int>& seg_rows) { int most = 0; for (int r : seg_rows) most = r > most ? r : most; return most; }
inline int small_level_strips(const lsfm_context* ctx, const std::vector<int>& seg_rows) { return small_level_strips(ctx, most_rows(seg_rows)); }
void small_level_offsets(lsfm_context* ctx, const DevBatch& out, SolveIO& io);
void small_solve_launch(lsfm_context* ctx, const SolveIO& io, int strips, int* status, double* max_rel);
struct HostSystem;
int small_selftest(lsfm_context* ctx, int G, const int* pose_off, const int* feat_off, const int* u_off, const unsigned char* active, const HostSystem& h,
                   const unsigned char* fixed, int strips, double* x_pose, double* x_feat, int* status, double* max_rel);
SolveOutcome solve_batch(lsfm_context* ctx, const SolveIO& io);
SolveOutcome join_batch_stereo(lsfm_context* ctx, Arena& ar, const DevBatch& in, DevBatch& out, double* eP_out, double* eF_out, int step_hint = 0);
SolveOutcome join_batch_mono(lsfm_context* ctx, Arena& ar, const DevBatch& in, DevBatch& out, double* eP_out, double* eF_out, int step_hint = 0);
int gn_polish(lsfm_context* ctx, const lsfm_map* maps, int N, bool mono, lsfm_map* x, int iters, int kind, double c, double* obj, double* gnorm,
              int* halvings, double* chi2, double* weight);
int map_feature_chi2(lsfm_context* ctx, const lsfm_map* maps, int N, bool mono, const lsfm_map* x, double* fchi2, double* pose_chi2);
int gn_polish_features(lsfm_context* ctx, const lsfm_map* maps, int N, bool mono, lsfm_map* x, int iters, int kind, double c, double* obj, double* gnorm,
                       int* halvings, double* fchi2, double* fweight);
int map_chi2(lsfm_context* ctx, const lsfm_map* maps, int N, bool mono, const lsfm_map* x, double* chi2, int* dof);
int gn_linearise(lsfm_context* ctx, const lsfm_map* maps, int N, bool mono, const lsfm_map* x, const double* weight, const double* fweight,
                 lsfm_map* out, double* obj, double* b, double* times, int* counts);
int map_covariance(lsfm_context* ctx, const lsfm_map* map, bool mono, double* pose_cov, double* feat_cov, double* pair_cov, int cap_blocks, int* nnzb,
                   double* times);
int map_covariance_columns(lsfm_context* ctx, const lsfm_map* map, bool mono, const int* poses, int k, double* pose_cols, double* feat_cols, double* joint,
                           int* steps, double* last_corr, double* times);
int map_covariance_feature_columns(lsfm_context* ctx, const lsfm_map* map, bool mono, const int* feats, int k, double* pose_cols, double* feat_cols,
                                   double* joint, int* steps, double* last_corr, double* times);
int map_feature_pair_gate(lsfm_context* ctx, const lsfm_map* map, bool mono, const int* pairs, int K, double* d2, double* cov_diff, int* steps,
                          double* last_corr, double* times);
int map_feature_pair_joint_gate(lsfm_context* ctx, const lsfm_map* map, bool mono, const int* pairs, int K, const int* order, double tau, int* status,
                                double* delta, double* d2, double* joint_C, int* accepted, int* implied, double* D2, int* steps, double* last_corr, double* times);
int pair_select_selftest(lsfm_context* ctx, int K, const double* C, const double* d, const int* ends, const int* order, double tau, int* status, double* delta,
                         double* D2, int* accepted, int* implied);
int map_merge_features(lsfm_context* ctx, const lsfm_map* map, bool mono, const int* pairs, int K, lsfm_map* out, double* d2, int* dof, int* rep,
                       int* steps, double* last_corr, double* times);
int map_feature_pair_candidates(lsfm_context* ctx, const lsfm_map* map, const double* feat_cov, double radius, double tau, int* pairs, double* dist2, double* q,
                                long long cap, long long* count, double* times, long long* info);
int inverse_v(lsfm_context* ctx, double* V, int n);
int vinv_selftest(lsfm_context* ctx, const double* V, const double* eb, int n, int skip, double* IV, double* LY);
int solve_features(lsfm_context* ctx, const double* W, const double* IV, const double* eb, const double* dpa, double* dpb, int m, int n, const int* mapCor,
                   const int* photo);
bool no_timing_events();
#define LSFM_REC_T(e, s) do { if (!lsfm::no_timing_events()) LSFM_CHECK_HIP(hipEventRecord(e, s)); } while (0)
unsigned timing_event_flags();
unsigned order_event_flags();
void prefetch_next_level(lsfm_context* ctx, const DevBatch& Y, const std::vector<int>& target_ref, int next_level, int step_hint,
                         const unsigned long long* level_keys, int level_nnzb);
int spmv_external(lsfm_context* ctx, int m, const int* rowptr, const int* colidx, const double* val, const double* x, double* y, int reps,
                  double* avg_ms, double* bytes);
int chol_selftest(lsfm_context* ctx, int m, const int* rowptr, const int* colidx, const double* val, const int* origin, const unsigned char* fixed,
                  const int* pose_seg, int nseg, const double* r, int nrhs, int mode, double* z, double* dot, int* perm, int* colptr, int* rowidx,
                  double* L, double* Dinv, double* dscale, int cap_blocks, int* info);
int cc_sweeps_selftest(lsfm_context* ctx, int m, const int* rowptr, const int* colidx, const double* val, const int* origin, const unsigned char* fixed,
                       const double* B, int R, const double* X, double* x, double* fwd, int* perm, double* dscale, double* y, int* info);

int wstream_bench(lsfm_context* ctx, long long nblocks, int mode, int reps, double* avg_ms);
int prims_selftest(lsfm_context* ctx, int cases, unsigned seed);
}
```

linearsfm_amd/csrc/lsfm_join.hip:

```cpp
#include "lsfm_device.hpp"
#include "lsfm_internal.hpp"
#include <climits>
#include "lsfm_join.hpp"
#include "lsfm_solve.hpp"

namespace lsfm {

__device__ __forceinline__ unsigned long long jh_mix(unsigned long long x)
{
	x ^= x >> 33; x *= 0xff51afd7ed558ccdull; x ^= x >> 33; x *= 0xc4ceb9fe1a85ec53ull; x ^= x >> 33;
	return x;
}
__global__ void k_join_hash_insert(int NF, const int* __restrict__ feat_id, const int* __restrict__ feat_map, unsigned long long* tab,
                                   int* __restrict__ tval, unsigned long long mask)
{
	int f = blockIdx.x * blockDim.x + threadIdx.x;
	if (f >= NF) return;
	const int mp = feat_map[f];
	if (mp & 1) return;
	const unsigned long long key = ((unsigned long long)(mp >> 1) << 32) | (unsigned)feat_id[f];
	unsigned long long h = jh_mix(key) & mask;
	for (;;)
	{
		const unsigned long long old = atomicCAS(&tab[h], ~0ull, key);
// ... 170 lines not shown
	__shared__ int ekeys[RHSU_CAP];
	__shared__ double evals[RHSU_CAP * 6];
	tile_clear<6>(ekeys, evals, RHSU_CAP);
	__syncthreads();
	const int i = blockIdx.x * blockDim.x + threadIdx.x;
	const bool have = i < NU;
	int a = 0, b = 0;
	double sa[6] = { 0, 0, 0, 0, 0, 0 }, sb[6] = { 0, 0, 0, 0, 0, 0 };
	if (have)
	{
		a = Ui[i]; b = Uj[i];
		double u[36];
		ld<36>(u, U + (size_t)i * 36);
		u_block_rhs(u, pose + (size_t)a * 6, pose + (size_t)b * 6, a != b, sa, sb);
	}
	tile_scatter_add<6>(ekeys, evals, RHSU_CAP, a, eP + (size_t)a * 6, sa, have);
	tile_scatter_add<6>(ekeys, evals, RHSU_CAP, b, eP + (size_t)b * 6, sb, have && a != b);
	__syncthreads();
	tile_flush<6>(ekeys, evals, RHSU_CAP, eP);
}

void join_layout(int B, const std::vector<int>& feat_off, const std::vector<int>& pose_off, const std::vector<int>& rb, int shared, DevBatch& out,
                 std::vector<JGroup>& grp, std::vector<int>& seg_rows, std::vector<unsigned char>& seg_active)
{
	const int G = (B + 1) / 2;
	out.feat_off.assign(G + 1, 0); out.pose_off.assign(G + 1, 0);
	grp.resize(G); seg_rows.assign(G, 0); seg_active.assign(G, 0);
	for (int g = 0; g < G; g++)
	{
		const int a = 2 * g, b = 2 * g + 1;
		const bool pair = b < B;
		JGroup& jg = grp[g];
		jg.F0E = feat_off[a]; jg.nE = feat_off[a + 1] - jg.F0E;
		jg.F0C = pair ? feat_off[b] : feat_off[a + 1]; jg.nC = pair ? feat_off[b + 1] - jg.F0C : 0;
		jg.FY0 = out.feat_off[g];
		jg.rC0 = pair ? rb[b] : 0;
		out.feat_off[g + 1] = jg.FY0 + jg.nE + (pair ? rb[b + 1] - rb[b] : 0);
		seg_active[g] = pair ? 1 : 0;
		seg_rows[g] = pair ? pose_off[b + 1] - pose_off[a] - shared : pose_off[a + 1] - pose_off[a];
		out.pose_off[g + 1] = out.pose_off[g] + seg_rows[g];
	}
}

SolveIO join_solve_io(lsfm_context* ctx, const DevBatch& out, const unsigned char* d_act, const double* eP, const double* eF,
                      const std::vector<int>& seg_rows, bool at_evA, int step_hint)
{
	SolveIO io;
	io.M = out.M; io.NF = out.NF; io.NU = out.NU; io.NW = out.NW; io.nseg = out.B;
	io.d_pose_seg = out.pose_map; io.d_feat_seg = out.feat_map; io.d_seg_active = d_act;
	io.U = out.U; io.Ui = out.Ui; io.Uj = out.Uj; io.W = out.W; io.photo = out.photo; io.fptr = out.fptr; io.V = out.V;
	io.ea = eP; io.eb = eF; io.d_pose_origin = out.pose_origin;
	io.x_pose = out.pose; io.x_feat = out.feat;
	io.seg_rows = seg_rows;
	io.index_arrays_at_evA = at_evA; io.step_hint = step_hint;
	small_level_offsets(ctx, out, io);
	return io;
}

void join_close(lsfm_context* ctx, size_t smark, const SolveOutcome& oc, bool whole_level)
{
	ctx->scratch.release(smark);
	if (oc.not_converged > 0 && ctx->stats) ctx->stats->not_converged += oc.not_converged;
	if (ctx->plan && whole_level) ctx->plan->valid = true;
}

void join_stereo_prepare(lsfm_context* ctx, Arena& ar, const DevBatch& in, DevBatch& out, JoinState& st, const DevBatch* level_in, const int* hub)
{
	hipStream_t s = ctx->stream;
	const int B = in.B, G = (B + 1) / 2;
	st.smark = ctx->scratch.mark();

	LevelPlan* plan = ctx->plan;
	const int *match = nullptr, *R = nullptr;
	const int nb = (in.NF + 255) / 256;
	std::vector<int> rb(B + 1);
	if (ctx->warm() && plan->idx.match && plan->idx.R && plan->idx.NF == in.NF)
	{
		match = plan->idx.match; R = plan->idx.R;
		rb = plan->join_rb;
	}
	else
	{
		const JoinRanks jr = join_rank_features(ctx, in);
		match = jr.match; R = jr.R;
		if (ctx->warm()) rb = plan->join_rb;
		else
		{
			int* d_rb = ctx->scratch.alloc<int>(B + 1);
			hipLaunchKernelGGL(k_gather_at, dim3((B + 1 + 127) / 128), dim3(128), 0, s, R, in.d_feat_off, B + 1, d_rb);
			ctx->mark("jn_enq");
			d2h_ints(ctx, d_rb, rb.data(), B + 1);
			ctx->mark("jn_rb");
			if (plan) plan->join_rb = rb;
			if (plan && plan != &ctx->pre_plan && ctx->in_tree_run)
			{
				plan->idx.match = level_index_keep(ctx, plan->idx, jr.match, (size_t)in.NF + 1);
				plan->idx.R = level_index_keep(ctx, plan->idx, jr.R, (size_t)in.NF + 2);
				plan->idx.NF = in.NF;
			}
		}
	}

	out = DevBatch();
	out.B = G; out.M = in.M; out.NU = in.NU; out.NW = in.NW;
	out.u_off.assign(G + 1, 0); out.w_off.assign(G + 1, 0);
	out.Ref.resize(G); out.FRef.resize(G); out.ScaP.assign(G, 0); out.Fix.assign(G, 0); out.Sign.assign(G, 1); out.FScaP.assign(G, 0); out.FFix.assign(G, 0);
	std::vector<JGroup> grp;
	std::vector<unsigned char>& seg_active = st.seg_active;
	std::vector<int>& seg_rows = st.seg_rows;
	join_layout(B, in.feat_off, in.pose_off, rb, 0, out, grp, seg_rows, seg_active);
	for (int g = 0; g < G; g++)
	{
		const int a = 2 * g, b = 2 * g + 1;
		out.u_off[g] = in.u_off[a]; out.w_off[g] = in.w_off[a];
		out.Ref[g] = b < B ? in.Ref[b] : in.Ref[a];
		out.FRef[g] = in.FRef[a];
	}
	out.u_off[G] = in.NU; out.w_off[G] = in.NW;
	out.NF = out.feat_off[G];
	const int NFY = out.NF;

	CopyBatch cb(ctx);
	JGroup* d_grp = ctx->scratch.alloc<JGroup>(G);
	cb.h2d(d_grp, grp.data(), sizeof(JGroup) * G);

	out.pose = ar.alloc<double>((size_t)in.M * 6);
	out.pose_id = ar.alloc<int>(in.M);
	out.pose_origin = ar.alloc<int>(in.M);
	cb.d2d(out.pose_origin, in.pose_origin, (size_t)in.M * sizeof(int));
	out.feat = ar.alloc<double>((size_t)NFY * 3);
	out.feat_id = ar.alloc<int>(NFY);
	out.U = ar.alloc<double>((size_t)in.NU * 36); out.Ui = ar.alloc<int>(in.NU); out.Uj = ar.alloc<int>(in.NU);
	out.W = ar.alloc<double>((size_t)in.NW * 18); out.photo = ar.alloc<int>(in.NW); out.feature = ar.alloc<int>(in.NW);
	out.fptr = ar.alloc<int>(NFY + 1);
	out.V = ar.alloc<double>((size_t)NFY * 9);
	batch_set_offsets(ctx, ar, out, &cb);
	cb.d2d(out.pose_id, in.pose_id, (size_t)in.M * sizeof(int));
	st.d_act = reinterpret_cast<unsigned char*>(ctx->scratch.alloc<int>((G + 3) / 4 + 1));
	st.act_padded.assign(((size_t)G + 3) / 4 * 4, 0);
	std::copy(seg_active.begin(), seg_active.end(), st.act_padded.begin());
	cb.h2d(st.d_act, st.act_padded.data(), st.act_padded.size());
	cb.flush();
	batch_fill_maps(ctx, out);
	int* newf = st.newf = ctx->scratch.alloc<int>(in.NF + 1);
	int* lens = ctx->scratch.alloc<int>(NFY + 2);
	st.srcf = ctx->scratch.alloc<int>(in.NW + 1);
	int* lenE = st.lenE = ctx->scratch.alloc<int>(NFY + 1);
	int* lenC = ctx->scratch.alloc<int>(NFY + 1);
	double* eF = st.eF = ctx->scratch.alloc<double>((size_t)NFY * 3);
	double* eP = st.eP = ctx->scratch.alloc<double>((size_t)in.M * 6);
	dev_zero(ctx, eP, (size_t)in.M * 6 * sizeof(double));
	const bool small_level = small_level_strips(ctx, seg_rows) > 0;
	const bool early = !small_level && !ctx->comm && !(ctx->pre && !ctx->pre_plan.valid) && level_in && hub && !ctx->warm() && level_in->NF == in.NF && level_in->M == in.M;
	st.fuse_rhs = !small_level && !ctx->comm && !ctx->pcg.mixed;
	int *srcE = nullptr, *srcC = nullptr;
	if (early || st.fuse_rhs)
	{
		srcE = ctx->scratch.alloc<int>(NFY + 1); srcC = ctx->scratch.alloc<int>(NFY + 1);
	}
	st.srcE = srcE; st.srcC = srcC;
	if (in.NF)
		for (int side = 0; side < 2; side++)
			hipLaunchKernelGGL(k_join_features, dim3(nb), dim3(256), 0, s, in.NF, in.feat_map, in.feat_id, in.feat, in.V, in.fptr, match, R, d_grp,
			                   newf, lenE, lenC, out.V, eF, out.feat_id, out.feat, srcE, srcC, side);
	if (early)
	{
		const DevBatch& X = *level_in;
		EarlyPatternIn ei;
		ei.M = in.M; ei.NFY = NFY; ei.NU = X.NU;
		ei.Ui = X.Ui; ei.Uj = X.Uj; ei.pose_map = X.pose_map; ei.hub = hub;
		ei.fptr = X.fptr; ei.photo = X.photo; ei.feat_map = X.feat_map; ei.srcE = srcE; ei.srcC = srcC;
		LSFM_CHECK_HIP(hipEventRecord(ctx->ord[evC_pairs], s));
		schur_pattern_early_issue(ctx, ei);
	}
	else schur_pattern_early_drop(ctx);
	hipLaunchKernelGGL(k_add_lens, dim3((NFY + 256) / 256), dim3(256), 0, s, NFY, lenE, lenC, lens);
	dev_exclusive_scan(ctx, lens, out.fptr, NFY);
	if (early) LSFM_CHECK_HIP(hipEventRecord(ctx->ord[evC_runs], s));
	st.wbase = ctx->scratch.alloc<int>(in.NF + 1);
	if (in.NF) hipLaunchKernelGGL(k_join_wbase, dim3(nb), dim3(256), 0, s, in.NF, in.feat_map, newf, lenE, out.fptr, st.wbase);
	LSFM_CHECK_HIP(hipGetLastError());
	ctx->mark("jn_prep");
}

SolveOutcome join_stereo_finish(lsfm_context* ctx, const DevBatch& in, DevBatch& out, JoinState& st, double* eP_out, double* eF_out, int step_hint)
{
	hipStream_t s = ctx->stream;
	const int NFY = out.NF;
	double *eP = st.eP, *eF = st.eF;
	int* srcf = st.srcf;
	if (in.NU)
	{
		CopyBatch cu(ctx);
		cu.d2d(out.U, in.U, (size_t)in.NU * 36 * sizeof(double));
		cu.d2d(out.Ui, in.Ui, (size_t)in.NU * sizeof(int));
		cu.d2d(out.Uj, in.Uj, (size_t)in.NU * sizeof(int));
		cu.flush();
	}
	LSFM_CHECK_HIP(hipEventRecord(ctx->ord[evY], s));
	const bool at_evA = !eP_out && !eF_out && !ctx->early && !ctx->comm;
	if (at_evA) LSFM_CHECK_HIP(hipEventRecord(ctx->ord[evA], s));
	const bool fuse_rhs = st.fuse_rhs && !eP_out && !eF_out;
	if (NFY && !fuse_rhs)
		hipLaunchKernelGGL(k_join_rhs_w, dim3((NFY + RHS_TILE - 1) / RHS_TILE), dim3(256), 0, s, NFY, out.fptr, out.W, out.photo, srcf, in.pose, in.feat, eP, eF);
	if (in.NU && (!ctx->comm || ctx->comm->rank == 0))
		hipLaunchKernelGGL(k_join_rhs_u, dim3((in.NU + 127) / 128), dim3(128), 0, s, in.NU, in.U, in.Ui, in.Uj, in.pose, eP);
	LSFM_CHECK_HIP(hipGetLastError());
	if (eP_out) d2h(ctx, eP_out, eP, (size_t)in.M * 6 * sizeof(double));
	if (eF_out) d2h(ctx, eF_out, eF, (size_t)NFY * 3 * sizeof(double));

	SolveIO io = join_solve_io(ctx, out, st.d_act, eP, eF, st.seg_rows, at_evA, step_hint);
	io.x0 = in.pose;
	RhsFused rhs;
	if (fuse_rhs)
	{
		rhs.srcE = st.srcE; rhs.srcC = st.srcC; rhs.feat_src = in.feat; rhs.pose_src = in.pose; rhs.pose_map_src = in.pose_map;
		io.rhs = &rhs;
	}
	const bool warm = ctx->warm();
	const SolveOutcome oc = solve_batch(ctx, io);
	if (!warm && !ctx->in_tree_run) LSFM_CHECK_HIP(hipStreamSynchronize(s));
	join_close(ctx, st.smark, oc, !eP_out && !eF_out);
	return oc;
}

SolveOutcome join_batch_stereo(lsfm_context* ctx, Arena& ar, const DevBatch& in, DevBatch& out, double* eP_out, double* eF_out, int step_hint)
{
	JoinState st;
	join_stereo_prepare(ctx, ar, in, out, st, nullptr, nullptr);
	if (in.NW)
		hipLaunchKernelGGL(k_join_wcopy, dim3((in.NW + 255) / 256), dim3(256), 0, ctx->stream, in.NW, in.W, in.photo, in.feature, in.fptr, st.wbase,
		                   st.newf, out.W, out.photo, out.feature, st.srcf, in.W_alias, in.d_alias, in.feat_map);
	return join_stereo_finish(ctx, in, out, st, eP_out, eF_out, step_hint);
}

}
```

linearsfm_amd/csrc/lsfm_small.hip:

```cpp
#include <algorithm>
#include <cstring>
#include <string>
#include <type_traits>

#include "lsfm_device.hpp"
#include "lsfm_internal.hpp"
#include "lsfm_solve.hpp"
#include "lsfm_system.hpp"

namespace lsfm {

#define SM_PASS 16
#define SM_K (3 * SM_PASS)
#define SM_KS (SM_K + 1)
#define SM_THREADS 256
#define SM_CHUNK 256
#define SM_SUPER 64
#define SM_WROWS 1024

typedef double sm_v4d __attribute__((ext_vector_type(4)));

struct SmallArgs {
	int nseg;
	const int *pose_off, *feat_off, *u_off;
	const unsigned char* seg_active;
	const double* U; const int *Ui, *Uj;
	const double* W; const int *photo, *fptr;
	const double* V;
	const double *ea, *eb, *x0;
	const unsigned char* fixed;
	double *x_pose, *x_feat;
	RunStatsDev* run;
	int* status;
	double* max_rel;
	int dbg;
};

template <int NTR>
struct SmallShared {
	static constexpr int R = 16 * NTR;
	double S[R * (R + 1)];
	double P[R * SM_KS];
	double d0[R];
	double E[R], x[R], r[R], v[R], dinv[R];
	double ly[SM_SUPER * 9];
	double wst[SM_WROWS * 3];
	int sph[SM_WROWS / 6 + 1];
	int fpc[2][SM_CHUNK + 1];
	unsigned char fx[R];
	int bad;
	int strips[4];
};

template <int NTR>
#ifndef LSFM_SMALL_OCC
#define LSFM_SMALL_OCC 2
#endif
__global__ void __launch_bounds__(SM_THREADS, NTR >= 6 ? 1 : (NTR <= 2 ? LSFM_SMALL_OCC : 2))
k_small_solve(SmallArgs a)
{
	constexpr int R = 16 * NTR, LD = R + 1;
	constexpr int NTILE = NTR * (NTR + 1) / 2, NW = SM_THREADS / 64, T = (NTILE + NW - 1) / NW;
	extern __shared__ double sm_raw[];
	SmallShared<NTR>& sh = *reinterpret_cast<SmallShared<NTR>*>(sm_raw);
	const int g = blockIdx.x, tid = threadIdx.x, lane = tid & 63, wave = __builtin_amdgcn_readfirstlane(tid >> 6);
	const int p0 = a.pose_off[g], m = a.pose_off[g + 1] - p0, n = 6 * m;
	const int f0 = a.feat_off[g], f1 = a.feat_off[g + 1];
	if (a.seg_active && !a.seg_active[g])
	{
		for (int i = tid; i < n; i += SM_THREADS) a.x_pose[(size_t)p0 * 6 + i] = a.x0 ? a.x0[(size_t)p0 * 6 + i] : 0.0;
		return;
	}
	for (int i = tid; i < R * LD; i += SM_THREADS) sh.S[i] = 0.0;
	for (int i = tid; i < R; i += SM_THREADS)
	{
		sh.E[i] = i < n ? a.ea[(size_t)p0 * 6 + i] : 0.0;
		sh.fx[i] = (i >= n || (a.fixed && a.fixed[(size_t)p0 * 6 + i])) ? 1 : 0;
	}
	if (tid == 0) sh.bad = 0;
	__syncthreads();
	{
		const int u0 = a.u_off[g], u1 = a.u_off[g + 1];
		for (int q = tid; q < (u1 - u0) * 36; q += SM_THREADS)
		{
			const int i = u0 + q / 36, e = q % 36, r = e / 6, c = e % 6;
			const int pa = a.Ui[i] - p0, pb = a.Uj[i] - p0;
			const double v = a.U[(size_t)i * 36 + e];
			lds_add_f64(&sh.S[(6 * pa + r) * LD + 6 * pb + c], v);
			if (pa != pb) lds_add_f64(&sh.S[(6 * pb + c) * LD + 6 * pa + r], v);
		}
	}
	int ti[T], tj[T];
	sm_v4d acc[T];
#pragma unroll
	for (int t = 0; t < T; t++)
	{
		const int q = wave + NW * t;
		int i = 0, j = 0;
		if (q < NTILE)
		{
			while ((j + 1) * (j + 2) / 2 <= q) j++;
			i = q - j * (j + 1) / 2;
		}
		ti[t] = q < NTILE ? i : -1; tj[t] = j;
		acc[t] = (sm_v4d){ 0.0, 0.0, 0.0, 0.0 };
	}
	constexpr int NE = (NTR + NW - 1) / NW;
	double eacc[NE];
#pragma unroll
	for (int i = 0; i < NE; i++) eacc[i] = 0.0;
	const int lbase = (lane & 15) * SM_KS + (lane >> 4);
	constexpr int PF = SM_WROWS / SM_THREADS;
	constexpr int MCAP = R / 6;
	double pw[PF][3];
	int pk[PF];
	double pv[9], pe[3];
	int qbn = 0, c0 = f0, cb = 1;
	auto prefetch = [&](int q0) {
		const int nf = min(SM_SUPER, f1 - q0);
		if (q0 - c0 >= SM_CHUNK || q0 == f0)
		{
			c0 = q0; cb ^= 1;
			for (int i = tid; i <= min(SM_CHUNK, f1 - c0); i += SM_THREADS) sh.fpc[cb][i] = a.fptr[c0 + i];
			__syncthreads();
		}
		qbn = sh.fpc[cb][q0 - c0];
		const int rw = (sh.fpc[cb][q0 - c0 + nf] - qbn) * 6;
		if (tid < nf)
		{
			ld<9>(pv, a.V + (size_t)(q0 + tid) * 9);
			ld<3>(pe, a.eb + (size_t)(q0 + tid) * 3);
		}
		const double* wb = a.W + (size_t)qbn * 18;
#pragma unroll
		for (int i = 0; i < PF; i++)
		{
			const int w = tid + SM_THREADS * i;
			if (w < rw) { pw[i][0] = wb[3 * (size_t)w]; pw[i][1] = wb[3 * (size_t)w + 1]; pw[i][2] = wb[3 * (size_t)w + 2]; pk[i] = a.photo[qbn + w / 6]; }
		}
	};
	for (int i = tid; i < R * SM_KS; i += SM_THREADS) sh.P[i] = 0.0;
	if (f0 < f1) prefetch(f0);
	for (int s0 = f0; s0 < f1; s0 += SM_SUPER)
	{
		const int nfs = min(SM_SUPER, f1 - s0);
		const int qbs = qbn, cs = c0, bs = cb;
		const int rws = (sh.fpc[bs][s0 - cs + nfs] - qbs) * 6;
		__syncthreads();
#pragma unroll
		for (int i = 0; i < PF; i++)
		{
			const int w = tid + SM_THREADS * i;
			if (w < rws)
			{
				sh.wst[3 * w] = pw[i][0]; sh.wst[3 * w + 1] = pw[i][1]; sh.wst[3 * w + 2] = pw[i][2];
				if (w % 6 == 0) sh.sph[w / 6] = pk[i] - p0;
			}
		}
		if (tid < 4) sh.strips[tid] = 0;
		if (tid < SM_SUPER)
		{
			double l[9];
#pragma unroll
			for (int i = 0; i < 9; i++) l[i] = 0.0;
			if (tid < nfs && !(a.dbg & 1))
			{
				double o[9];
				inv3_sym(pv, o);
				const double d0 = o[0];
				l[0] = sqrt(d0); l[1] = o[3] / l[0]; l[3] = o[6] / l[0];
				const double d1 = o[4] - l[1] * l[1];
				l[2] = sqrt(d1); l[4] = (o[7] - l[3] * l[1]) / l[2];
				const double d2 = o[8] - l[3] * l[3] - l[4] * l[4];
				l[5] = sqrt(d2);
				l[6] = l[0] * pe[0] + l[1] * pe[1] + l[3] * pe[2];
				l[7] = l[2] * pe[1] + l[4] * pe[2];
				l[8] = l[5] * pe[2];
				if (!(d0 > 0.0) || !(d1 > 0.0) || !(d2 > 0.0)) sh.bad = 1;
			}
			st<9>(&sh.ly[tid * 9], l);
		}
		__syncthreads();
		if (s0 + SM_SUPER < f1) prefetch(s0 + SM_SUPER);
		for (int sub = 0; sub * SM_PASS < nfs; sub++)
		{
			const int q0 = s0 + sub * SM_PASS, nf = min(SM_PASS, f1 - q0);
			{
				const int lp = tid >> 4, fl = tid & 15;
				bool found = false;
				if (lp < MCAP && !(a.dbg & 2))
				{
					double c18[18];
#pragma unroll
					for (int i = 0; i < 18; i++) c18[i] = 0.0;
					if (fl < nf && lp < m)
					{
						const int j0 = sh.fpc[bs][q0 - cs + fl], j1 = sh.fpc[bs][q0 - cs + fl + 1];
						const double* l = &sh.ly[(sub * SM_PASS + fl) * 9];
						const double l0 = l[0], l1 = l[1], l2 = l[2], l3 = l[3], l4 = l[4], l5 = l[5];
						for (int j = j0; j < j1; j++)
						{
							const int e = j - qbs;
							const int ph = 6 * e < SM_WROWS ? sh.sph[e] : a.photo[j] - p0;
							if (ph != lp) continue;
							found = true;
#pragma unroll
							for (int r = 0; r < 6; r++)
							{
								double w0, w1, w2;
								if (6 * e + 5 < SM_WROWS) { w0 = sh.wst[3 * (6 * e + r)]; w1 = sh.wst[3 * (6 * e + r) + 1]; w2 = sh.wst[3 * (6 * e + r) + 2]; }
								else { const double* wg = a.W + (size_t)j * 18 + 3 * r; w0 = wg[0]; w1 = wg[1]; w2 = wg[2]; }
								c18[3 * r] += w0 * l0 + w1 * l1 + w2 * l3;
								c18[3 * r + 1] += w1 * l2 + w2 * l4;
								c18[3 * r + 2] += w2 * l5;
							}
						}
					}
#pragma unroll
					for (int r = 0; r < 6; r++)
					{
						double* d = &sh.P[(6 * lp + r) * SM_KS + 3 * fl];
						d[0] = c18[3 * r]; d[1] = c18[3 * r + 1]; d[2] = c18[3 * r + 2];
					}
				}
				const int b0 = (6 * lp) >> 4, b1 = (6 * lp + 5) >> 4;
#pragma unroll
				for (int sidx = 0; sidx < NTR; sidx++)
					if (__ballot(found && (b0 == sidx || b1 == sidx)) != 0ull && lane == 0) atomicOr(&sh.strips[sub], 1 << sidx);
			}
			__syncthreads();
			const int smask = sh.strips[sub];
			{
				const int kq = lane >> 4;
#pragma unroll
				for (int si = 0; si < NE; si++)
				{
					const int strip = wave + NW * si;
					if (strip < NTR && ((smask >> strip) & 1) && !(a.dbg & 4))
					{
						const double* pr = &sh.P[(16 * strip + (lane & 15)) * SM_KS + 12 * kq];
						const double* yq = &sh.ly[sub * SM_PASS * 9 + kq * 36 + 6];
						double e0 = 0.0, e1 = 0.0;
#pragma unroll
						for (int k = 0; k < 12; k += 2)
						{
							e0 = fma(pr[k], yq[(k / 3) * 9 + k % 3], e0);
							e1 = fma(pr[k + 1], yq[((k + 1) / 3) * 9 + (k + 1) % 3], e1);
						}
						double sum = e0 + e1;
						sum += __shfl_xor(sum, 16, 64);
						sum += __shfl_xor(sum, 32, 64);
						eacc[si] -= sum;
					}
				}
			}
			bool on[T];
#pragma unroll
			for (int t = 0; t < T; t++) on[t] = ti[t] >= 0 && (((smask >> ti[t]) & (smask >> tj[t]) & 1) != 0) && !(a.dbg & 8);
#pragma unroll 2
			for (int ks = 0; ks < SM_K / 4; ks++)
			{
#pragma unroll
				for (int t = 0; t < T; t++)
				{
					if (!on[t]) continue;
					const double av = sh.P[16 * ti[t] * SM_KS + lbase + 4 * ks], bv = sh.P[16 * tj[t] * SM_KS + lbase + 4 * ks];
					acc[t] = __builtin_amdgcn_mfma_f64_16x16x4f64(av, bv, acc[t], 0, 0, 0);
				}
			}
			__syncthreads();
		}
	}
	__syncthreads();
#pragma unroll
	for (int t = 0; t < T; t++)
	{
		if (ti[t] < 0) continue;
		const int C = 16 * tj[t] + (lane & 15);
#pragma unroll
		for (int e = 0; e < 4; e++)
		{
			const int Rr = 16 * ti[t] + (lane >> 4) + 4 * e;
			const double v = acc[t][e];
			sh.S[Rr * LD + C] -= v;
			if (ti[t] != tj[t]) sh.S[C * LD + Rr] -= v;
		}
	}
	if (lane < 16)
#pragma unroll
		for (int si = 0; si < NE; si++)
		{
			const int strip = wave + NW * si;
			if (strip < NTR) sh.E[16 * strip + lane] += eacc[si];
		}
	__syncthreads();
	for (int q = tid; q < R * R; q += SM_THREADS)
	{
		const int i = q / R, j = q - i * R;
		if (sh.fx[i] || sh.fx[j]) sh.S[i * LD + j] = i == j ? 1.0 : 0.0;
	}
	for (int i = tid; i < R; i += SM_THREADS) if (sh.fx[i]) sh.E[i] = 0.0;
	__syncthreads();
	for (int i = tid; i < R; i += SM_THREADS) sh.d0[i] = sh.S[i * LD + i];
	__syncthreads();
	int pivot_bad = -1;
	for (int j = 0; j < ((a.dbg & 16) ? 0 : n); j++)
	{
		const double d = sh.S[j * LD + j];
		if (!(d > 0.0) || !(d < 1e300)) { pivot_bad = j; break; }
		const double piv = sqrt(d), ip = 1.0 / piv;
		__syncthreads();
		for (int i = j + tid; i < n; i += SM_THREADS) sh.S[i * LD + j] = i == j ? piv : sh.S[i * LD + j] * ip;
		__syncthreads();
		{
			const int ty = tid >> 4, tx = tid & 15;
			for (int i = j + 1 + ty; i < n; i += 16)
			{
				const double lij = sh.S[i * LD + j];
				for (int k = j + 1 + tx; k <= i; k += 16) sh.S[i * LD + k] = fma(-lij, sh.S[k * LD + j], sh.S[i * LD + k]);
			}
		}
		__syncthreads();
	}
	if (pivot_bad >= 0)
	{
		if (tid == 0) { atomicCAS(&a.status[1], 0, 1 + g); if (a.run && !a.run->chol_err) a.run->chol_err = 1 + p0 + pivot_bad / 6; }
		return;
	}
	for (int i = tid; i < n; i += SM_THREADS) sh.dinv[i] = 1.0 / sh.S[i * LD + i];
	__syncthreads();
	auto solve = [&](const double* rhs, double* out) {
		for (int i = tid; i < R; i += SM_THREADS) sh.v[i] = i < n ? rhs[i] : 0.0;
		__syncthreads();
		if (wave == 0)
		{
			for (int j = 0; j < n; j++)
			{
				const double vj = sh.v[j] * sh.dinv[j];
				__builtin_amdgcn_wave_barrier();
				if (lane == 0) sh.v[j] = vj;
				for (int i = j + 1 + lane; i < n; i += 64) sh.v[i] = fma(-sh.S[i * LD + j], vj, sh.v[i]);
				__builtin_amdgcn_wave_barrier();
			}
			for (int j = n - 1; j >= 0; j--)
			{
				const double vj = sh.v[j] * sh.dinv[j];
				__builtin_amdgcn_wave_barrier();
				if (lane == 0) sh.v[j] = vj;
				for (int i = lane; i < j; i += 64) sh.v[i] = fma(-sh.S[j * LD + i], vj, sh.v[i]);
				__builtin_amdgcn_wave_barrier();
			}
		}
		__syncthreads();
		for (int i = tid; i < R; i += SM_THREADS) out[i] = sh.v[i];
		__syncthreads();
	};
	auto residual = [&](const double* xx) {
		for (int i = tid; i < n; i += SM_THREADS)
		{
			double s = sh.E[i] - sh.d0[i] * xx[i];
			for (int j = 0; j < n; j++)
				if (j != i) s = fma(-(i < j ? sh.S[i * LD + j] : sh.S[j * LD + i]), xx[j], s);
			sh.r[i] = s;
		}
		__syncthreads();
	};
	if (!(a.dbg & 16))
	{
	solve(sh.E, sh.x);
	residual(sh.x);
	solve(sh.r, sh.v);
	for (int i = tid; i < n; i += SM_THREADS) sh.x[i] += sh.v[i];
	__syncthreads();
	residual(sh.x);
	}
	if (tid == 0)
	{
		double rr = 0.0, ee = 0.0;
		for (int i = 0; i < n; i++) { rr += sh.r[i] * sh.r[i]; ee += sh.E[i] * sh.E[i]; }
		const double rel = ee > 0.0 ? sqrt(rr / ee) : 0.0;
		if (!(rel < 1e-8) || sh.bad)
		{
			atomicAdd(&a.status[0], 1);
			if (a.run) atomicAdd(&a.run->not_converged, 1);
		}
		const unsigned long long bits = (unsigned long long)__double_as_longlong(rel == rel ? rel : 1e300);
		atomicMax(reinterpret_cast<unsigned long long*>(a.max_rel), bits);
		if (a.run) atomicMax(reinterpret_cast<unsigned long long*>(&a.run->max_rel_residual), bits);
	}
	for (int i = tid; i < n; i += SM_THREADS) a.x_pose[(size_t)p0 * 6 + i] = sh.fx[i] ? 0.0 : sh.x[i];
	for (int f = f0 + tid; f < ((a.dbg & 32) ? f0 : f1); f += SM_THREADS)
	{
		double V[9], iv[9];
		ld<9>(V, a.V + (size_t)f * 9);
		inv3_sym(V, iv);
		double d[3] = { a.eb[(size_t)f * 3], a.eb[(size_t)f * 3 + 1], a.eb[(size_t)f * 3 + 2] };
		double s3[3] = { 0.0, 0.0, 0.0 };
		for (int j = a.fptr[f]; j < a.fptr[f + 1]; j++)
		{
			double w[18];
			ld<18>(w, a.W + (size_t)j * 18);
			const double* xp = &sh.x[6 * (a.photo[j] - p0)];
#pragma unroll
			for (int c = 0; c < 3; c++)
			{
				double sacc = 0.0;
#pragma unroll
				for (int r = 0; r < 6; r++) sacc = fma(w[3 * r + c], sh.fx[6 * (a.photo[j] - p0) + r] ? 0.0 : xp[r], sacc);
				s3[c] += sacc;
			}
		}
		d[0] -= s3[0]; d[1] -= s3[1]; d[2] -= s3[2];
		for (int r = 0; r < 3; r++) a.x_feat[(size_t)f * 3 + r] = iv[3 * r] * d[0] + iv[3 * r + 1] * d[1] + iv[3 * r + 2] * d[2];
	}
}

static int small_solve_strips(int most_poses, int cap)
{
	if (most_poses > cap) return 0;
	if (most_poses <= 2) return 1;
	if (most_poses <= 5) return 2;
	if (most_poses <= 8) return 3;
	if (most_poses <= 16) return 6;
	return 0;
}
int small_level_strips(const lsfm_context* ctx, int most_rows)
{
	return (ctx->small_max > 0 && !ctx->comm && !ctx->pcg.mixed) ? small_solve_strips(most_rows, ctx->small_max) : 0;
}
void small_level_offsets(lsfm_context* ctx, const DevBatch& out, SolveIO& io)
{
	if (!small_level_strips(ctx, io.seg_rows)) return;
	const int G = io.nseg;
	int* d_uo = ctx->scratch.alloc<int>(G + 1);
	h2d(ctx, d_uo, out.u_off.data(), sizeof(int) * (size_t)(G + 1));
	io.d_pose_off = out.d_pose_off; io.d_feat_off = out.d_feat_off; io.d_u_off = d_uo;
}

template <int NTR>
static void launch_small(hipStream_t s, const SmallArgs& a)
{
	const size_t lds = sizeof(SmallShared<NTR>);
	static const bool set = []() {
		(void)hipFuncSetAttribute(reinterpret_cast<const void*>(&k_small_solve<NTR>), hipFuncAttributeMaxDynamicSharedMemorySize, (int)sizeof(SmallShared<NTR>));
		return true;
	}();
	(void)set;
	hipLaunchKernelGGL(k_small_solve<NTR>, dim3(a.nseg), dim3(SM_THREADS), lds, s, a);
}

void small_solve_launch(lsfm_context* ctx, const SolveIO& io, int strips, int* status, double* max_rel)
{
	SmallArgs a;
	a.nseg = io.nseg; a.pose_off = io.d_pose_off; a.feat_off = io.d_feat_off; a.u_off = io.d_u_off; a.seg_active = io.d_seg_active;
	a.U = io.U; a.Ui = io.Ui; a.Uj = io.Uj; a.W = io.W; a.photo = io.photo; a.fptr = io.fptr; a.V = io.V;
	a.ea = io.ea; a.eb = io.eb; a.x0 = io.x0; a.fixed = io.d_fixed; a.x_pose = io.x_pose; a.x_feat = io.x_feat;
	a.run = (ctx->in_tree_run && ctx->d_run) ? ctx->d_run : nullptr;
	a.status = status; a.max_rel = max_rel;
	a.dbg = getenv("LSFM_SMALL_DEBUG") ? atoi(getenv("LSFM_SMALL_DEBUG")) : 0;
	if (!io.nseg) return;
	switch (strips)
	{
	case 1: launch_small<1>(ctx->stream, a); break;
	case 2: launch_small<2>(ctx->stream, a); break;
	case 3: launch_small<3>(ctx->stream, a); break;
	default: launch_small<6>(ctx->stream, a); break;
	}
	LSFM_CHECK_HIP(hipGetLastError());
}

int small_selftest(lsfm_context* ctx, int G, const int* pose_off, const int* feat_off, const int* u_off, const unsigned char* active, const HostSystem& h,
                   const unsigned char* fixed, int strips, double* x_pose, double* x_feat, int* status, double* max_rel)
{
	if (pose_off[0] || feat_off[0] || u_off[0] || pose_off[G] != h.m || feat_off[G] != h.n || u_off[G] != h.nU)
		LSFM_FAIL(LSFM_ERR_ARG, "the offsets must run from 0 to the batch's poses / features / U blocks");
	const std::vector<int> fptr = system_fptr(h);
	int most = 0;
	for (int g = 0; g < G; g++)
	{
		const int p0 = pose_off[g], p1 = pose_off[g + 1];
		if (p1 <= p0 || feat_off[g + 1] < feat_off[g] || u_off[g + 1] < u_off[g]) LSFM_FAIL(LSFM_ERR_ARG, "system " + std::to_string(g) + ": empty or negative range");
		most = std::max(most, p1 - p0);
		for (int i = u_off[g]; i < u_off[g + 1]; i++)
			if (h.Ui[i] < p0 || h.Uj[i] >= p1) LSFM_FAIL(LSFM_ERR_ARG, "system " + std::to_string(g) + ": a U block of another system's pose");
		for (int j = fptr[feat_off[g]]; j < fptr[feat_off[g + 1]]; j++)
			if (h.photo[j] < p0 || h.photo[j] >= p1) LSFM_FAIL(LSFM_ERR_ARG, "system " + std::to_string(g) + ": a W block of another system's pose");
	}
	if (most > 16) LSFM_FAIL(LSFM_ERR_ARG, "a system of " + std::to_string(most) + " poses: the dense path holds 16");
	if (!strips) strips = small_solve_strips(most, 16);
	if (strips != 1 && strips != 2 && strips != 3 && strips != 6) LSFM_FAIL(LSFM_ERR_ARG, "strips must be 0, 1, 2, 3 or 6");
	if (6 * most > 16 * strips) LSFM_FAIL(LSFM_ERR_ARG, "a system of " + std::to_string(most) + " poses does not fit a panel of " + std::to_string(strips) + " strips");
	SolveIO io;
	system_upload(ctx, h, SYS_VALUES | SYS_RHS | SYS_X, fptr, nullptr, io);
	Arena& ar = ctx->arena[0];
	auto up = [&](auto* src, size_t count) {
		auto* d = ar.alloc<std::remove_cv_t<std::remove_pointer_t<decltype(src)>>>(count);
		h2d(ctx, d, src, count * sizeof *src);
		return d;
	};
	io.nseg = G;
	io.d_pose_off = up(pose_off, (size_t)G + 1); io.d_feat_off = up(feat_off, (size_t)G + 1); io.d_u_off = up(u_off, (size_t)G + 1);
	if (active) io.d_seg_active = up(active, (size_t)G);
	if (fixed) io.d_fixed = up(fixed, (size_t)h.m * 6);
	h2d(ctx, io.x_pose, x_pose, (size_t)h.m * 6 * sizeof(double));
	h2d(ctx, io.x_feat, x_feat, (size_t)h.n * 3 * sizeof(double));
	int* d_small = ctx->scratch.alloc<int>(4);
	dev_zero(ctx, d_small, 4 * sizeof(int));
	small_solve_launch(ctx, io, strips, d_small, reinterpret_cast<double*>(d_small + 2));
	int hs[4];
	d2h_ints(ctx, d_small, hs, 4);
	status[0] = hs[0]; status[1] = hs[1];
	memcpy(max_rel, hs + 2, sizeof *max_rel);
	d2h(ctx, x_pose, io.x_pose, (size_t)h.m * 6 * sizeof(double));
	d2h(ctx, x_feat, io.x_feat, (size_t)h.n * 3 * sizeof(double));
	return LSFM_OK;
}

}
```

Before: 29.58.

## Fuse join right-hand-side build into the small dense solve kernel

Enables the fused right-hand side on small-level joins, so the small dense per-segment solver reads source indices and previous estimates and folds the RHS correction into its feature pass. A separate RHS construction pass and its memory traffic are no longer needed. For small strip counts, each wave now accumulates its own partial P panel, and the camera system reuses the shared memory that held the W rows, which lowers LDS footprint. This adds per-lane triangular solves and extra index loads, and aliasing the system onto the W-row buffer is a correctness risk.

```diff
diff --git a/include/lsfm.h b/include/lsfm.h
--- a/include/lsfm.h
+++ b/include/lsfm.h
@@ -251,6 +251,12 @@
                         const double* ea, const double* eb, const double* x0, const unsigned char* fixed, int strips, double* x_pose, double* x_feat,
                         int* status, double* max_rel);
 
+int lsfm_selftest_small_rhs(lsfm_context* ctx, int G, const int* pose_off, const int* feat_off, const int* u_off, const unsigned char* active,
+                            const double* U, const int* Ui, const int* Uj, const double* W, const int* photo, const int* feature, int nW, const double* V,
+                            const double* ea, const double* eb, const double* x0, const unsigned char* fixed, int strips, const double* pose_est,
+                            const unsigned char* pose_side, const double* feat_end, const double* feat_cur, const unsigned char* has_end,
+                            const unsigned char* has_cur, double* x_pose, double* x_feat, int* status, double* max_rel);
+
 #ifdef __cplusplus
 }
 #endif
diff --git a/linearsfm_amd/api.py b/linearsfm_amd/api.py
--- a/linearsfm_amd/api.py
+++ b/linearsfm_amd/api.py
@@ -171,6 +171,8 @@
         L.lsfm_selftest_cc_sweeps.argtypes = [vp, C.c_int, ip, ip, dp, ip, P(C.c_ubyte), dp, C.c_int, dp, dp, dp, ip, dp, dp, ip]
         L.lsfm_selftest_transform.argtypes = [vp, P(LsfmMap), C.c_int, C.c_int, ip, ip, ip, C.c_int, P(LsfmMap)]
         L.lsfm_selftest_small.argtypes = [vp, C.c_int, ip, ip, ip, ub, dp, ip, ip, dp, ip, ip, C.c_int, dp, dp, dp, dp, ub, C.c_int, dp, dp, ip, dp]
+        L.lsfm_selftest_small_rhs.argtypes = [vp, C.c_int, ip, ip, ip, ub, dp, ip, ip, dp, ip, ip, C.c_int, dp, dp, dp, dp, ub, C.c_int, dp, ub, dp, dp, ub, ub,
+                                              dp, dp, ip, dp]
         _LIB = L
     return _LIB
 
@@ -183,7 +185,7 @@
            "lsfm_tree_free", "lsfm_divide_conquer", "lsfm_read_localmap", "lsfm_read_localmaps", "lsfm_write_localmap", "lsfm_write_mapset", "lsfm_mapset_info", "lsfm_mapset_stamp", "lsfm_read_mapset", "lsfm_save_state_bin", "lsfm_save_state", "lsfm_save_poses", "lsfm_gn_polish",
            "lsfm_gn_polish_robust", "lsfm_map_chi2", "lsfm_map_feature_chi2", "lsfm_gn_polish_robust_features", "lsfm_gn_linearise", "lsfm_gn_linearise_timed",
            "lsfm_gn_linearise_features", "lsfm_gn_linearise_features_timed",
-           "lsfm_spmv_bench", "lsfm_wstream_bench", "lsfm_selftest_prims", "lsfm_selftest_chol", "lsfm_selftest_cc_sweeps", "lsfm_selftest_transform", "lsfm_selftest_small", "lsfm_schur_pattern", "lsfm_symbolic_analyse", "lsfm_inverse_v", "lsfm_selftest_vinv", "lsfm_solve_features",
+           "lsfm_spmv_bench", "lsfm_wstream_bench", "lsfm_selftest_prims", "lsfm_selftest_chol", "lsfm_selftest_cc_sweeps", "lsfm_selftest_transform", "lsfm_selftest_small", "lsfm_selftest_small_rhs", "lsfm_schur_pattern", "lsfm_symbolic_analyse", "lsfm_inverse_v", "lsfm_selftest_vinv", "lsfm_solve_features",
            "lsfm_map_covariance", "lsfm_map_covariance_timed",
            "lsfm_save_covariances", "lsfm_read_covariances",
            "lsfm_map_covariance_columns", "lsfm_map_covariance_columns_timed", "lsfm_save_cov_columns", "lsfm_read_cov_columns",
@@ -933,7 +935,7 @@
 Context.selftest_transform = _selftest_transform
 
 
-def _selftest_small(self, B, strips=0, active=None, fixed=None, x0=None, prefill=None):
+def _selftest_small(self, B, strips=0, active=None, fixed=None, x0=None, prefill=None, rhs=None):
     po, fo, uo = (_c(B[k], np.int32) for k in ("pose_off", "feat_off", "u_off"))
     G = len(po) - 1
     if G < 1 or len(fo) != G + 1 or len(uo) != G + 1:
@@ -955,6 +957,16 @@
     st = np.zeros(2, np.int32)
     mr = C.c_double()
     d, i, opt = C.c_double, C.c_int, lambda a, t: None if a is None else _ptr(a, t)
+    if rhs is not None:
+        pe = _fit(_c(rhs["pose_est"], np.float64), 6 * M, "pose_est")
+        fe_, fc_ = (_fit(_c(rhs[k], np.float64), 3 * NF, k) for k in ("feat_end", "feat_cur"))
+        ps, he, hc = flags(rhs["pose_side"], M, "pose_side"), flags(rhs["has_end"], NF, "has_end"), flags(rhs["has_cur"], NF, "has_cur")
+        rc = lib().lsfm_selftest_small_rhs(self._h, G, _ptr(po, i), _ptr(fo, i), _ptr(uo, i), opt(act, C.c_ubyte), _ptr(U, d), _ptr(Ui, i), _ptr(Uj, i),
+                                           _ptr(W, d), _ptr(ph, i), _ptr(fe, i), nW, _ptr(V, d), _ptr(ea, d), _ptr(eb, d), opt(x0, d), opt(fx, C.c_ubyte),
+                                           int(strips), _ptr(pe, d), _ptr(ps, C.c_ubyte), _ptr(fe_, d), _ptr(fc_, d), _ptr(he, C.c_ubyte), _ptr(hc, C.c_ubyte),
+                                           _ptr(xp, d), _ptr(xf, d), _ptr(st, i), C.byref(mr))
+        self._check(rc, "lsfm_selftest_small_rhs")
+        return xp, xf, st, mr.value
     rc = lib().lsfm_selftest_small(self._h, G, _ptr(po, i), _ptr(fo, i), _ptr(uo, i), opt(act, C.c_ubyte), _ptr(U, d), _ptr(Ui, i), _ptr(Uj, i),
                                    _ptr(W, d), _ptr(ph, i), _ptr(fe, i), nW, _ptr(V, d), _ptr(ea, d), _ptr(eb, d), opt(x0, d), opt(fx, C.c_ubyte),
                                    int(strips), _ptr(xp, d), _ptr(xf, d), _ptr(st, i), C.byref(mr))
@@ -969,6 +981,7 @@
 
 
 Context.selftest_small = _selftest_small
+Context.selftest_small_rhs = lambda self, B, rhs, **kw: _selftest_small(self, B, rhs=rhs, **kw)
 
 
 def symbolic_analyse(rowptr, colidx, origin=None, reps=1):
diff --git a/linearsfm_amd/csrc/lsfm_capi.hip b/linearsfm_amd/csrc/lsfm_capi.hip
--- a/linearsfm_amd/csrc/lsfm_capi.hip
+++ b/linearsfm_amd/csrc/lsfm_capi.hip
@@ -814,6 +814,28 @@
 	});
 }
 
+int lsfm_selftest_small_rhs(lsfm_context* ctx, int G, const int* pose_off, const int* feat_off, const int* u_off, const unsigned char* active,
+                            const double* U, const int* Ui, const int* Uj, const double* W, const int* photo, const int* feature, int nW, const double* V,
+                            const double* ea, const double* eb, const double* x0, const unsigned char* fixed, int strips, const double* pose_est,
+                            const unsigned char* pose_side, const double* feat_end, const double* feat_cur, const unsigned char* has_end,
+                            const unsigned char* has_cur, double* x_pose, double* x_feat, int* status, double* max_rel)
+{
+	if (G <= 0 || !pose_off || !feat_off || !u_off || !ea || !x_pose || !status || !max_rel || strips < 0 || nW < 0 || !pose_est || !pose_side) return LSFM_ERR_ARG;
+	const int M = pose_off[G], NF = feat_off[G], NU = u_off[G];
+	if (M <= 0 || NF < 0 || NU < 0 || (NU && (!U || !Ui || !Uj)) || (nW && (!W || !photo || !feature)) || (NF && (!V || !eb || !x_feat))) return LSFM_ERR_ARG;
+	if (NF && (!feat_end || !feat_cur || !has_end || !has_cur)) return LSFM_ERR_ARG;
+	status[0] = status[1] = 0; *max_rel = 0.0;
+	return guarded(ctx, [&]() {
+		HostSystem h;
+		h.m = M; h.n = NF; h.nU = NU; h.nW = nW;
+		h.Ui = Ui; h.Uj = Uj; h.photo = photo; h.feature = feature;
+		h.U = U; h.W = W; h.V = V; h.ea = ea; h.eb = eb; h.x0 = x0;
+		SmallRhsHost r;
+		r.pose_est = pose_est; r.pose_side = pose_side; r.feat_end = feat_end; r.feat_cur = feat_cur; r.has_end = has_end; r.has_cur = has_cur;
+		return small_selftest(ctx, G, pose_off, feat_off, u_off, active, h, fixed, strips, x_pose, x_feat, status, max_rel, &r);
+	});
+}
+
 int lsfm_wstream_bench(lsfm_context* ctx, long long nblocks, int mode, int reps, double* avg_ms)
 {
 	if (nblocks <= 0 || mode < 0 || mode > 2 || reps <= 0 || !avg_ms) return LSFM_ERR_ARG;
diff --git a/linearsfm_amd/csrc/lsfm_internal.hpp b/linearsfm_amd/csrc/lsfm_internal.hpp
--- a/linearsfm_amd/csrc/lsfm_internal.hpp
+++ b/linearsfm_amd/csrc/lsfm_internal.hpp
@@ -393,8 +393,14 @@
 void small_level_offsets(lsfm_context* ctx, const DevBatch& out, SolveIO& io);
 void small_solve_launch(lsfm_context* ctx, const SolveIO& io, int strips, int* status, double* max_rel);
 struct HostSystem;
+struct SmallRhsHost {
+	const double* pose_est = nullptr;
+	const unsigned char* pose_side = nullptr;
+	const double *feat_end = nullptr, *feat_cur = nullptr;
+	const unsigned char *has_end = nullptr, *has_cur = nullptr;
+};
 int small_selftest(lsfm_context* ctx, int G, const int* pose_off, const int* feat_off, const int* u_off, const unsigned char* active, const HostSystem& h,
-                   const unsigned char* fixed, int strips, double* x_pose, double* x_feat, int* status, double* max_rel);
+                   const unsigned char* fixed, int strips, double* x_pose, double* x_feat, int* status, double* max_rel, const SmallRhsHost* rhs = nullptr);
 SolveOutcome solve_batch(lsfm_context* ctx, const SolveIO& io);
 SolveOutcome join_batch_stereo(lsfm_context* ctx, Arena& ar, const DevBatch& in, DevBatch& out, double* eP_out, double* eF_out, int step_hint = 0);
 SolveOutcome join_batch_mono(lsfm_context* ctx, Arena& ar, const DevBatch& in, DevBatch& out, double* eP_out, double* eF_out, int step_hint = 0);
diff --git a/linearsfm_amd/csrc/lsfm_join.hip b/linearsfm_amd/csrc/lsfm_join.hip
--- a/linearsfm_amd/csrc/lsfm_join.hip
+++ b/linearsfm_amd/csrc/lsfm_join.hip
@@ -346,7 +346,7 @@
 	dev_zero(ctx, eP, (size_t)in.M * 6 * sizeof(double));
 	const bool small_level = small_level_strips(ctx, seg_rows) > 0;
 	const bool early = !small_level && !ctx->comm && !(ctx->pre && !ctx->pre_plan.valid) && level_in && hub && !ctx->warm() && level_in->NF == in.NF && level_in->M == in.M;
-	st.fuse_rhs = !small_level && !ctx->comm && !ctx->pcg.mixed;
+	st.fuse_rhs = !ctx->comm && !ctx->pcg.mixed;
 	int *srcE = nullptr, *srcC = nullptr;
 	if (early || st.fuse_rhs)
 	{
diff --git a/linearsfm_amd/csrc/lsfm_small.hip b/linearsfm_amd/csrc/lsfm_small.hip
--- a/linearsfm_amd/csrc/lsfm_small.hip
+++ b/linearsfm_amd/csrc/lsfm_small.hip
@@ -29,6 +29,9 @@
 	const double* V;
 	const double *ea, *eb, *x0;
 	const unsigned char* fixed;
+	const int *srcE, *srcC;
+	const double *feat_src, *pose_src;
+	const int* pose_map_src;
 	double *x_pose, *x_feat;
 	RunStatsDev* run;
 	int* status;
@@ -37,19 +40,34 @@
 };
 
 template <int NTR>
+struct SmallSystem {
+	static constexpr int R = 16 * NTR;
+	double S[R * (R + 1)];
+	double d0[R];
+	double E[R], x[R], r[R], v[R], dinv[R];
+	double xh[R];
+	unsigned char fx[R];
+};
+struct SmallNone {};
+template <int NTR>
 struct SmallShared {
 	static constexpr int R = 16 * NTR;
-	double S[R * (R + 1)];
-	double P[R * SM_KS];
-	double d0[R];
-	double E[R], x[R], r[R], v[R], dinv[R];
-	double ly[SM_SUPER * 9];
+	static constexpr bool WP = NTR <= 2;
+	static constexpr int NP = WP ? SM_SUPER / SM_PASS : 1, PR = NTR == 2 ? 30 : R;
+	std::conditional_t<WP, SmallNone, SmallSystem<NTR>> own;
+	double P[NP * PR * SM_KS];
+	double ly[SM_SUPER * 6];
+	double yu[SM_SUPER * 6];
 	double wst[SM_WROWS * 3];
 	int sph[SM_WROWS / 6 + 1];
 	int fpc[2][SM_CHUNK + 1];
-	unsigned char fx[R];
 	int bad;
 	int strips[4];
+	__device__ SmallSystem<NTR>& system()
+	{
+		if constexpr (WP) { static_assert(sizeof(SmallSystem<NTR>) <= sizeof(wst), "the camera system lies where the W rows were"); return *reinterpret_cast<SmallSystem<NTR>*>(wst); }
+		else return own;
+	}
 };
 
 template <int NTR>
@@ -63,33 +81,41 @@
 	constexpr int NTILE = NTR * (NTR + 1) / 2, NW = SM_THREADS / 64, T = (NTILE + NW - 1) / NW;
 	extern __shared__ double sm_raw[];
 	SmallShared<NTR>& sh = *reinterpret_cast<SmallShared<NTR>*>(sm_raw);
+	SmallSystem<NTR>& po = sh.system();
+	constexpr bool WP = SmallShared<NTR>::WP;
+	constexpr int PR = SmallShared<NTR>::PR, PSZ = PR * SM_KS;
 	const int g = blockIdx.x, tid = threadIdx.x, lane = tid & 63, wave = __builtin_amdgcn_readfirstlane(tid >> 6);
 	const int p0 = a.pose_off[g], m = a.pose_off[g + 1] - p0, n = 6 * m;
 	const int f0 = a.feat_off[g], f1 = a.feat_off[g + 1];
+	const bool fused = a.srcE != nullptr;
 	if (a.seg_active && !a.seg_active[g])
 	{
 		for (int i = tid; i < n; i += SM_THREADS) a.x_pose[(size_t)p0 * 6 + i] = a.x0 ? a.x0[(size_t)p0 * 6 + i] : 0.0;
 		return;
 	}
-	for (int i = tid; i < R * LD; i += SM_THREADS) sh.S[i] = 0.0;
-	for (int i = tid; i < R; i += SM_THREADS)
-	{
-		sh.E[i] = i < n ? a.ea[(size_t)p0 * 6 + i] : 0.0;
-		sh.fx[i] = (i >= n || (a.fixed && a.fixed[(size_t)p0 * 6 + i])) ? 1 : 0;
-	}
 	if (tid == 0) sh.bad = 0;
-	__syncthreads();
-	{
-		const int u0 = a.u_off[g], u1 = a.u_off[g + 1];
-		for (int q = tid; q < (u1 - u0) * 36; q += SM_THREADS)
-		{
-			const int i = u0 + q / 36, e = q % 36, r = e / 6, c = e % 6;
-			const int pa = a.Ui[i] - p0, pb = a.Uj[i] - p0;
-			const double v = a.U[(size_t)i * 36 + e];
-			lds_add_f64(&sh.S[(6 * pa + r) * LD + 6 * pb + c], v);
-			if (pa != pb) lds_add_f64(&sh.S[(6 * pb + c) * LD + 6 * pa + r], v);
-		}
-	}
+	auto system_begin = [&]() {
+		for (int i = tid; i < R * LD; i += SM_THREADS) po.S[i] = 0.0;
+		for (int i = tid; i < R; i += SM_THREADS)
+		{
+			po.E[i] = i < n ? a.ea[(size_t)p0 * 6 + i] : 0.0;
+			po.fx[i] = (i >= n || (a.fixed && a.fixed[(size_t)p0 * 6 + i])) ? 1 : 0;
+			po.xh[i] = (fused && i < n) ? a.pose_src[(size_t)p0 * 6 + i] : 0.0;
+		}
+		__syncthreads();
+		{
+			const int u0 = a.u_off[g], u1 = a.u_off[g + 1];
+			for (int q = tid; q < (u1 - u0) * 36; q += SM_THREADS)
+			{
+				const int i = u0 + q / 36, e = q % 36, r = e / 6, c = e % 6;
+				const int pa = a.Ui[i] - p0, pb = a.Uj[i] - p0;
+				const double v = a.U[(size_t)i * 36 + e];
+				lds_add_f64(&po.S[(6 * pa + r) * LD + 6 * pb + c], v);
+				if (pa != pb) lds_add_f64(&po.S[(6 * pb + c) * LD + 6 * pa + r], v);
+			}
+		}
+	};
+	if constexpr (!WP) system_begin();
 	int ti[T], tj[T];
 	sm_v4d acc[T];
 #pragma unroll
@@ -109,15 +135,50 @@
 	double eacc[NE];
 #pragma unroll
 	for (int i = 0; i < NE; i++) eacc[i] = 0.0;
+	int eside[NE];
+#pragma unroll
+	for (int i = 0; i < NE; i++)
+	{
+		const int pose = (16 * (wave + NW * i) + (lane & 15)) / 6;
+		eside[i] = (fused && pose < m && (a.pose_map_src[p0 + pose] & 1)) ? 3 : 0;
+	}
 	const int lbase = (lane & 15) * SM_KS + (lane >> 4);
+	constexpr int NWA = WP ? NTILE : 1, NWE = WP ? NTR : 1;
+	sm_v4d wacc[NWA];
+	int wrow[NWE];
+	double weacc[NWE];
+	int wside[NWE];
+#pragma unroll
+	for (int q = 0; q < NWA; q++) wacc[q] = (sm_v4d){ 0.0, 0.0, 0.0, 0.0 };
+#pragma unroll
+	for (int i = 0; i < NWE; i++)
+	{
+		const int pose = (16 * i + (lane & 15)) / 6;
+		weacc[i] = 0.0;
+		wrow[i] = min(16 * i + (lane & 15), PR - 1) * SM_KS + (lane >> 4);
+		wside[i] = (fused && pose < m && (a.pose_map_src[p0 + pose] & 1)) ? 3 : 0;
+	}
 	constexpr int PF = SM_WROWS / SM_THREADS;
 	constexpr int MCAP = R / 6;
 	double pw[PF][3];
 	int pk[PF];
 	double pv[9], pe[3];
+	double px[6];
+	bool hasE = false, hasC = false;
+	int nsE = -1, nsC = -1;
+	if (fused && tid < min(SM_SUPER, f1 - f0)) { nsE = a.srcE[f0 + tid]; nsC = a.srcC[f0 + tid]; }
 	int qbn = 0, c0 = f0, cb = 1;
 	auto prefetch = [&](int q0) {
 		const int nf = min(SM_SUPER, f1 - q0);
+		if (fused && tid < SM_SUPER)
+		{
+			const int sE = nsE, sC = nsC;
+			nsE = nsC = -1;
+			if (q0 + SM_SUPER + tid < f1) { nsE = a.srcE[q0 + SM_SUPER + tid]; nsC = a.srcC[q0 + SM_SUPER + tid]; }
+			hasE = sE >= 0; hasC = sC >= 0;
+			if (hasE) ld<3>(px, a.feat_src + (size_t)sE * 3);
+			if (hasC) ld<3>(px + 3, a.feat_src + (size_t)sC * 3);
+		}
 		if (q0 - c0 >= SM_CHUNK || q0 == f0)
 		{
 			c0 = q0; cb ^= 1;
@@ -139,7 +200,7 @@
 			if (w < rw) { pw[i][0] = wb[3 * (size_t)w]; pw[i][1] = wb[3 * (size_t)w + 1]; pw[i][2] = wb[3 * (size_t)w + 2]; pk[i] = a.photo[qbn + w / 6]; }
 		}
 	};
-	for (int i = tid; i < R * SM_KS; i += SM_THREADS) sh.P[i] = 0.0;
+	for (int i = tid; i < SmallShared<NTR>::NP * PSZ; i += SM_THREADS) sh.P[i] = 0.0;
 	if (f0 < f1) prefetch(f0);
 	for (int s0 = f0; s0 < f1; s0 += SM_SUPER)
 	{
@@ -178,10 +239,128 @@
 				l[8] = l[5] * pe[2];
 				if (!(d0 > 0.0) || !(d1 > 0.0) || !(d2 > 0.0)) sh.bad = 1;
 			}
-			st<9>(&sh.ly[tid * 9], l);
+			st<6>(&sh.ly[tid * 6], l);
+			double yu[6];
+#pragma unroll
+			for (int sd = 0; sd < 2; sd++)
+			{
+				double u0 = 0.0, u1 = 0.0, u2 = 0.0;
+				if (fused && tid < nfs && (sd ? hasC : hasE))
+				{
+					const double* x = px + 3 * sd;
+					u0 = x[0] / l[0];
+					u1 = (x[1] - l[1] * u0) / l[2];
+					u2 = (x[2] - l[3] * u0 - l[4] * u1) / l[5];
+				}
+				yu[3 * sd] = l[6] - u0; yu[3 * sd + 1] = l[7] - u1; yu[3 * sd + 2] = l[8] - u2;
+			}
+			st<6>(&sh.yu[tid * 6], yu);
 		}
 		__syncthreads();
 		if (s0 + SM_SUPER < f1) prefetch(s0 + SM_SUPER);
+		if constexpr (WP)
+		{
+			const int sub = wave;
+			if (sub * SM_PASS < nfs)
+			{
+				const int q0 = s0 + sub * SM_PASS, nf = min(SM_PASS, f1 - q0);
+				double* Pw = sh.P + wave * PSZ;
+				int smask = 0;
+				constexpr int ROUNDS = (32 * MCAP + 63) / 64;
+#pragma unroll
+				for (int rd = 0; rd < ROUNDS; rd++)
+				{
+					const int u = lane + 64 * rd, fl = u & 15, hf = (u >> 4) & 1, lp = u >> 5;
+					bool found = false;
+					if (lp < MCAP && !(a.dbg & 2))
+					{
+						double c9[9];
+#pragma unroll
+						for (int i = 0; i < 9; i++) c9[i] = 0.0;
+						if (fl < nf && lp < m)
+						{
+							const int j0 = sh.fpc[bs][q0 - cs + fl], j1 = sh.fpc[bs][q0 - cs + fl + 1];
+							const double* l = &sh.ly[(sub * SM_PASS + fl) * 6];
+							const double l0 = l[0], l1 = l[1], l2 = l[2], l3 = l[3], l4 = l[4], l5 = l[5];
+							for (int j = j0; j < j1; j++)
+							{
+								const int e = j - qbs;
+								const bool parked = 6 * e + 5 < SM_WROWS;
+								if ((parked ? sh.sph[e] : a.photo[j] - p0) != lp) continue;
+								found = true;
+#pragma unroll
+								for (int r = 0; r < 3; r++)
+								{
+									const int row = 6 * e + 3 * hf + r;
+									double w0, w1, w2;
+									if (parked) { w0 = sh.wst[3 * row]; w1 = sh.wst[3 * row + 1]; w2 = sh.wst[3 * row + 2]; }
+									else { const double* wg = a.W + (size_t)j * 18 + 3 * (3 * hf + r); w0 = wg[0]; w1 = wg[1]; w2 = wg[2]; }
+									c9[3 * r] += w0 * l0 + w1 * l1 + w2 * l3;
+									c9[3 * r + 1] += w1 * l2 + w2 * l4;
+									c9[3 * r + 2] += w2 * l5;
+								}
+							}
+						}
+#pragma unroll
+						for (int r = 0; r < 3; r++)
+						{
+							double* d = &Pw[(6 * lp + 3 * hf + r) * SM_KS + 3 * fl];
+							d[0] = c9[3 * r]; d[1] = c9[3 * r + 1]; d[2] = c9[3 * r + 2];
+						}
+					}
+					const int b0 = (6 * lp) >> 4, b1 = (6 * lp + 5) >> 4;
+#pragma unroll
+					for (int sidx = 0; sidx < NTR; sidx++)
+						if (__ballot(found && (b0 == sidx || b1 == sidx)) != 0ull) smask |= 1 << sidx;
+				}
+				__builtin_amdgcn_fence(__ATOMIC_RELEASE, "wavefront");
+				__builtin_amdgcn_wave_barrier();
+				__builtin_amdgcn_fence(__ATOMIC_ACQUIRE, "wavefront");
+				{
+					const int kq = lane >> 4;
+#pragma unroll
+					for (int strip = 0; strip < NTR; strip++)
+					{
+						if (((smask >> strip) & 1) && !(a.dbg & 4))
+						{
+							const double* pr = &Pw[min(16 * strip + (lane & 15), PR - 1) * SM_KS + 12 * kq];
+							const double* yq = &sh.yu[sub * SM_PASS * 6 + kq * 24 + wside[strip]];
+							double e0 = 0.0, e1 = 0.0;
+#pragma unroll
+							for (int k = 0; k < 12; k += 2)
+							{
+								e0 = fma(pr[k], yq[(k / 3) * 6 + k % 3], e0);
+								e1 = fma(pr[k + 1], yq[((k + 1) / 3) * 6 + (k + 1) % 3], e1);
+							}
+							double sum = e0 + e1;
+							sum += __shfl_xor(sum, 16, 64);
+							sum += __shfl_xor(sum, 32, 64);
+							weacc[strip] -= sum;
+						}
+					}
+				}
+				if (!(a.dbg & 8))
+				{
+#pragma unroll 2
+					for (int ks = 0; ks < SM_K / 4; ks++)
+					{
+#pragma unroll
+						for (int j = 0; j < NTR; j++)
+#pragma unroll
+							for (int i = 0; i <= j; i++)
+							{
+								if (!((smask >> i) & (smask >> j) & 1)) continue;
+								double av = Pw[wrow[i] + 4 * ks], bv = Pw[wrow[j] + 4 * ks];
+								if (PR < R && i == NTR - 1 && (lane & 15) >= PR - 16 * i) av = 0.0;
+								if (PR < R && j == NTR - 1 && (lane & 15) >= PR - 16 * j) bv = 0.0;
+								wacc[j * (j + 1) / 2 + i] = __builtin_amdgcn_mfma_f64_16x16x4f64(av, bv, wacc[j * (j + 1) / 2 + i], 0, 0, 0);
+							}
+					}
+				}
+				__builtin_amdgcn_wave_barrier();
+			}
+		}
+		else
 		for (int sub = 0; sub * SM_PASS < nfs; sub++)
 		{
 			const int q0 = s0 + sub * SM_PASS, nf = min(SM_PASS, f1 - q0);
@@ -196,7 +375,7 @@
 					if (fl < nf && lp < m)
 					{
 						const int j0 = sh.fpc[bs][q0 - cs + fl], j1 = sh.fpc[bs][q0 - cs + fl + 1];
-						const double* l = &sh.ly[(sub * SM_PASS + fl) * 9];
+						const double* l = &sh.ly[(sub * SM_PASS + fl) * 6];
 						const double l0 = l[0], l1 = l[1], l2 = l[2], l3 = l[3], l4 = l[4], l5 = l[5];
 						for (int j = j0; j < j1; j++)
 						{
@@ -239,13 +418,13 @@
 					if (strip < NTR && ((smask >> strip) & 1) && !(a.dbg & 4))
 					{
 						const double* pr = &sh.P[(16 * strip + (lane & 15)) * SM_KS + 12 * kq];
-						const double* yq = &sh.ly[sub * SM_PASS * 9 + kq * 36 + 6];
+						const double* yq = &sh.yu[sub * SM_PASS * 6 + kq * 24 + eside[si]];
 						double e0 = 0.0, e1 = 0.0;
 #pragma unroll
 						for (int k = 0; k < 12; k += 2)
 						{
-							e0 = fma(pr[k], yq[(k / 3) * 9 + k % 3], e0);
-							e1 = fma(pr[k + 1], yq[((k + 1) / 3) * 9 + (k + 1) % 3], e1);
+							e0 = fma(pr[k], yq[(k / 3) * 6 + k % 3], e0);
+							e1 = fma(pr[k + 1], yq[((k + 1) / 3) * 6 + (k + 1) % 3], e1);
 						}
 						double sum = e0 + e1;
 						sum += __shfl_xor(sum, 16, 64);
@@ -272,52 +451,122 @@
 		}
 	}
 	__syncthreads();
-#pragma unroll
-	for (int t = 0; t < T; t++)
-	{
-		if (ti[t] < 0) continue;
-		const int C = 16 * tj[t] + (lane & 15);
+	auto flush_tile = [&](const sm_v4d& av, int i, int j) {
+		const int C = 16 * j + (lane & 15);
 #pragma unroll
 		for (int e = 0; e < 4; e++)
 		{
-			const int Rr = 16 * ti[t] + (lane >> 4) + 4 * e;
-			const double v = acc[t][e];
-			sh.S[Rr * LD + C] -= v;
-			if (ti[t] != tj[t]) sh.S[C * LD + Rr] -= v;
-		}
-	}
-	if (lane < 16)
-#pragma unroll
-		for (int si = 0; si < NE; si++)
-		{
-			const int strip = wave + NW * si;
-			if (strip < NTR) sh.E[16 * strip + lane] += eacc[si];
-		}
+			const int Rr = 16 * i + (lane >> 4) + 4 * e;
+			po.S[Rr * LD + C] -= av[e];
+			if (i != j) po.S[C * LD + Rr] -= av[e];
+		}
+	};
+	auto tile_times_xh = [&](const sm_v4d& av, int i, int j, double* ax) {
+		const int C = 16 * j + (lane & 15);
+		double colsum = 0.0;
+#pragma unroll
+		for (int e = 0; e < 4; e++)
+		{
+			const int Rr = 16 * i + (lane >> 4) + 4 * e;
+			double rs = av[e] * po.xh[C];
+#pragma unroll
+			for (int o = 1; o < 16; o <<= 1) rs += __shfl_xor(rs, o, 64);
+			if ((lane & 15) == 0) ax[(lane >> 4) + 4 * e] = rs;
+			colsum = fma(av[e], po.xh[Rr], colsum);
+		}
+		if (i != j)
+		{
+			colsum += __shfl_xor(colsum, 16, 64);
+			colsum += __shfl_xor(colsum, 32, 64);
+			if (lane < 16) ax[16 + lane] = colsum;
+		}
+	};
+	if constexpr (WP)
+	{
+		system_begin();
+		__syncthreads();
+		if (fused)
+#pragma unroll
+			for (int j = 0; j < NTR; j++)
+#pragma unroll
+				for (int i = 0; i <= j; i++) tile_times_xh(wacc[j * (j + 1) / 2 + i], i, j, &sh.P[wave * PSZ + (j * (j + 1) / 2 + i) * 32]);
+		for (int w = 0; w < NW; w++)
+		{
+			if (wave == w)
+			{
+#pragma unroll
+				for (int j = 0; j < NTR; j++)
+#pragma unroll
+					for (int i = 0; i <= j; i++) flush_tile(wacc[j * (j + 1) / 2 + i], i, j);
+				if (lane < 16)
+#pragma unroll
+					for (int strip = 0; strip < NTR; strip++) po.E[16 * strip + lane] += weacc[strip];
+			}
+			__syncthreads();
+		}
+	}
+	else
+	{
+#pragma unroll
+		for (int t = 0; t < T; t++)
+		{
+			if (ti[t] < 0) continue;
+			flush_tile(acc[t], ti[t], tj[t]);
+			if (fused) tile_times_xh(acc[t], ti[t], tj[t], &sh.P[(wave + NW * t) * 32]);
+		}
+		if (lane < 16)
+#pragma unroll
+			for (int si = 0; si < NE; si++)
+			{
+				const int strip = wave + NW * si;
+				if (strip < NTR) po.E[16 * strip + lane] += eacc[si];
+			}
+		__syncthreads();
+	}
+	for (int q = tid; q < R * R; q += SM_THREADS)
+	{
+		const int i = q / R, j = q - i * R;
+		if (po.fx[i] || po.fx[j]) po.S[i * LD + j] = i == j ? 1.0 : 0.0;
+	}
+	for (int i = tid; i < R; i += SM_THREADS)
+	{
+		if (fused)
+		{
+			const int s = i >> 4, r = i & 15;
+			double ax = 0.0;
+#pragma unroll
+			for (int w = 0; w < SmallShared<NTR>::NP; w++)
+#pragma unroll
+				for (int j = 0; j < NTR; j++)
+#pragma unroll
+					for (int ii = 0; ii <= j; ii++)
+					{
+						const double* part = &sh.P[w * PSZ + (j * (j + 1) / 2 + ii) * 32];
+						if (ii == s) ax += part[r];
+						else if (j == s) ax += part[16 + r];
+					}
+			po.E[i] -= ax;
+		}
+		if (po.fx[i]) po.E[i] = 0.0;
+	}
 	__syncthreads();
-	for (int q = tid; q < R * R; q += SM_THREADS)
-	{
-		const int i = q / R, j = q - i * R;
-		if (sh.fx[i] || sh.fx[j]) sh.S[i * LD + j] = i == j ? 1.0 : 0.0;
-	}
-	for (int i = tid; i < R; i += SM_THREADS) if (sh.fx[i]) sh.E[i] = 0.0;
-	__syncthreads();
-	for (int i = tid; i < R; i += SM_THREADS) sh.d0[i] = sh.S[i * LD + i];
+	for (int i = tid; i < R; i += SM_THREADS) po.d0[i] = po.S[i * LD + i];
 	__syncthreads();
 	int pivot_bad = -1;
 	for (int j = 0; j < ((a.dbg & 16) ? 0 : n); j++)
 	{
-		const double d = sh.S[j * LD + j];
+		const double d = po.S[j * LD + j];
 		if (!(d > 0.0) || !(d < 1e300)) { pivot_bad = j; break; }
 		const double piv = sqrt(d), ip = 1.0 / piv;
 		__syncthreads();
-		for (int i = j + tid; i < n; i += SM_THREADS) sh.S[i * LD + j] = i == j ? piv : sh.S[i * LD + j] * ip;
+		for (int i = j + tid; i < n; i += SM_THREADS) po.S[i * LD + j] = i == j ? piv : po.S[i * LD + j] * ip;
 		__syncthreads();
 		{
 			const int ty = tid >> 4, tx = tid & 15;
 			for (int i = j + 1 + ty; i < n; i += 16)
 			{
-				const double lij = sh.S[i * LD + j];
-				for (int k = j + 1 + tx; k <= i; k += 16) sh.S[i * LD + k] = fma(-lij, sh.S[k * LD + j], sh.S[i * LD + k]);
+				const double lij = po.S[i * LD + j];
+				for (int k = j + 1 + tx; k <= i; k += 16) po.S[i * LD + k] = fma(-lij, po.S[k * LD + j], po.S[i * LD + k]);
 			}
 		}
 		__syncthreads();
@@ -327,57 +576,57 @@
 		if (tid == 0) { atomicCAS(&a.status[1], 0, 1 + g); if (a.run && !a.run->chol_err) a.run->chol_err = 1 + p0 + pivot_bad / 6; }
 		return;
 	}
-	for (int i = tid; i < n; i += SM_THREADS) sh.dinv[i] = 1.0 / sh.S[i * LD + i];
+	for (int i = tid; i < n; i += SM_THREADS) po.dinv[i] = 1.0 / po.S[i * LD + i];
 	__syncthreads();
 	auto solve = [&](const double* rhs, double* out) {
-		for (int i = tid; i < R; i += SM_THREADS) sh.v[i] = i < n ? rhs[i] : 0.0;
+		for (int i = tid; i < R; i += SM_THREADS) po.v[i] = i < n ? rhs[i] : 0.0;
 		__syncthreads();
 		if (wave == 0)
 		{
 			for (int j = 0; j < n; j++)
 			{
-				const double vj = sh.v[j] * sh.dinv[j];
+				const double vj = po.v[j] * po.dinv[j];
 				__builtin_amdgcn_wave_barrier();
-				if (lane == 0) sh.v[j] = vj;
-				for (int i = j + 1 + lane; i < n; i += 64) sh.v[i] = fma(-sh.S[i * LD + j], vj, sh.v[i]);
+				if (lane == 0) po.v[j] = vj;
+				for (int i = j + 1 + lane; i < n; i += 64) po.v[i] = fma(-po.S[i * LD + j], vj, po.v[i]);
 				__builtin_amdgcn_wave_barrier();
 			}
 			for (int j = n - 1; j >= 0; j--)
 			{
-				const double vj = sh.v[j] * sh.dinv[j];
+				const double vj = po.v[j] * po.dinv[j];
 				__builtin_amdgcn_wave_barrier();
-				if (lane == 0) sh.v[j] = vj;
-				for (int i = lane; i < j; i += 64) sh.v[i] = fma(-sh.S[j * LD + i], vj, sh.v[i]);
+				if (lane == 0) po.v[j] = vj;
+				for (int i = lane; i < j; i += 64) po.v[i] = fma(-po.S[j * LD + i], vj, po.v[i]);
 				__builtin_amdgcn_wave_barrier();
 			}
 		}
 		__syncthreads();
-		for (int i = tid; i < R; i += SM_THREADS) out[i] = sh.v[i];
+		for (int i = tid; i < R; i += SM_THREADS) out[i] = po.v[i];
 		__syncthreads();
 	};
 	auto residual = [&](const double* xx) {
 		for (int i = tid; i < n; i += SM_THREADS)
 		{
-			double s = sh.E[i] - sh.d0[i] * xx[i];
+			double s = po.E[i] - po.d0[i] * xx[i];
 			for (int j = 0; j < n; j++)
-				if (j != i) s = fma(-(i < j ? sh.S[i * LD + j] : sh.S[j * LD + i]), xx[j], s);
-			sh.r[i] = s;
+				if (j != i) s = fma(-(i < j ? po.S[i * LD + j] : po.S[j * LD + i]), xx[j], s);
+			po.r[i] = s;
 		}
 		__syncthreads();
 	};
 	if (!(a.dbg & 16))
 	{
-	solve(sh.E, sh.x);
-	residual(sh.x);
-	solve(sh.r, sh.v);
-	for (int i = tid; i < n; i += SM_THREADS) sh.x[i] += sh.v[i];
+	solve(po.E, po.x);
+	residual(po.x);
+	solve(po.r, po.v);
+	for (int i = tid; i < n; i += SM_THREADS) po.x[i] += po.v[i];
 	__syncthreads();
-	residual(sh.x);
+	residual(po.x);
 	}
 	if (tid == 0)
 	{
 		double rr = 0.0, ee = 0.0;
-		for (int i = 0; i < n; i++) { rr += sh.r[i] * sh.r[i]; ee += sh.E[i] * sh.E[i]; }
+		for (int i = 0; i < n; i++) { rr += po.r[i] * po.r[i]; ee += po.E[i] * po.E[i]; }
 		const double rel = ee > 0.0 ? sqrt(rr / ee) : 0.0;
 		if (!(rel < 1e-8) || sh.bad)
 		{
@@ -388,7 +637,14 @@
 		atomicMax(reinterpret_cast<unsigned long long*>(a.max_rel), bits);
 		if (a.run) atomicMax(reinterpret_cast<unsigned long long*>(&a.run->max_rel_residual), bits);
 	}
-	for (int i = tid; i < n; i += SM_THREADS) a.x_pose[(size_t)p0 * 6 + i] = sh.fx[i] ? 0.0 : sh.x[i];
+	for (int i = tid; i < n; i += SM_THREADS) a.x_pose[(size_t)p0 * 6 + i] = po.fx[i] ? 0.0 : po.x[i];
+	if (fused)
+	{
+		__syncthreads();
+		for (int i = tid; i < R; i += SM_THREADS) po.r[i] = (po.fx[i] ? 0.0 : po.x[i]) - po.xh[i];
+		__syncthreads();
+	}
+	const double* xs = fused ? po.r : po.x;
 	for (int f = f0 + tid; f < ((a.dbg & 32) ? f0 : f1); f += SM_THREADS)
 	{
 		double V[9], iv[9];
@@ -400,13 +656,13 @@
 		{
 			double w[18];
 			ld<18>(w, a.W + (size_t)j * 18);
-			const double* xp = &sh.x[6 * (a.photo[j] - p0)];
+			const double* xp = &xs[6 * (a.photo[j] - p0)];
 #pragma unroll
 			for (int c = 0; c < 3; c++)
 			{
 				double sacc = 0.0;
 #pragma unroll
-				for (int r = 0; r < 6; r++) sacc = fma(w[3 * r + c], sh.fx[6 * (a.photo[j] - p0) + r] ? 0.0 : xp[r], sacc);
+				for (int r = 0; r < 6; r++) sacc = fma(w[3 * r + c], (!fused && po.fx[6 * (a.photo[j] - p0) + r]) ? 0.0 : xp[r], sacc);
 				s3[c] += sacc;
 			}
 		}
@@ -455,6 +711,13 @@
 	a.nseg = io.nseg; a.pose_off = io.d_pose_off; a.feat_off = io.d_feat_off; a.u_off = io.d_u_off; a.seg_active = io.d_seg_active;
 	a.U = io.U; a.Ui = io.Ui; a.Uj = io.Uj; a.W = io.W; a.photo = io.photo; a.fptr = io.fptr; a.V = io.V;
 	a.ea = io.ea; a.eb = io.eb; a.x0 = io.x0; a.fixed = io.d_fixed; a.x_pose = io.x_pose; a.x_feat = io.x_feat;
+	a.srcE = a.srcC = a.pose_map_src = nullptr; a.feat_src = a.pose_src = nullptr;
+	if (io.rhs)
+	{
+		const RhsFused& r = *io.rhs;
+		if (!r.srcE || !r.srcC || !r.feat_src || !r.pose_src || !r.pose_map_src) LSFM_FAIL(LSFM_ERR_ARG, "a fused right-hand side without its sources");
+		a.srcE = r.srcE; a.srcC = r.srcC; a.feat_src = r.feat_src; a.pose_src = r.pose_src; a.pose_map_src = r.pose_map_src;
+	}
 	a.run = (ctx->in_tree_run && ctx->d_run) ? ctx->d_run : nullptr;
 	a.status = status; a.max_rel = max_rel;
 	a.dbg = getenv("LSFM_SMALL_DEBUG") ? atoi(getenv("LSFM_SMALL_DEBUG")) : 0;
@@ -470,7 +733,7 @@
 }
 
 int small_selftest(lsfm_context* ctx, int G, const int* pose_off, const int* feat_off, const int* u_off, const unsigned char* active, const HostSystem& h,
-                   const unsigned char* fixed, int strips, double* x_pose, double* x_feat, int* status, double* max_rel)
+                   const unsigned char* fixed, int strips, double* x_pose, double* x_feat, int* status, double* max_rel, const SmallRhsHost* rhs)
 {
 	if (pose_off[0] || feat_off[0] || u_off[0] || pose_off[G] != h.m || feat_off[G] != h.n || u_off[G] != h.nU)
 		LSFM_FAIL(LSFM_ERR_ARG, "the offsets must run from 0 to the batch's poses / features / U blocks");
@@ -502,6 +765,24 @@
 	io.d_pose_off = up(pose_off, (size_t)G + 1); io.d_feat_off = up(feat_off, (size_t)G + 1); io.d_u_off = up(u_off, (size_t)G + 1);
 	if (active) io.d_seg_active = up(active, (size_t)G);
 	if (fixed) io.d_fixed = up(fixed, (size_t)h.m * 6);
+	RhsFused fr;
+	if (rhs)
+	{
+		std::vector<int> srcE(h.n + 1, -1), srcC(h.n + 1, -1), side(h.m);
+		std::vector<double> fsrc((size_t)h.n * 6 + 1, 0.0);
+		for (int f = 0; f < h.n; f++)
+		{
+			if (rhs->has_end[f]) { srcE[f] = f; std::copy(rhs->feat_end + 3 * (size_t)f, rhs->feat_end + 3 * (size_t)f + 3, fsrc.begin() + 3 * (size_t)f); }
+			if (rhs->has_cur[f]) { srcC[f] = h.n + f; std::copy(rhs->feat_cur + 3 * (size_t)f, rhs->feat_cur + 3 * (size_t)f + 3, fsrc.begin() + 3 * (size_t)(h.n + f)); }
+		}
+		for (int p = 0; p < h.m; p++) side[p] = rhs->pose_side[p] ? 1 : 0;
+		fr.srcE = up(srcE.data(), srcE.size()); fr.srcC = up(srcC.data(), srcC.size());
+		fr.feat_src = up(fsrc.data(), fsrc.size());
+		fr.pose_src = up(rhs->pose_est, (size_t)h.m * 6);
+		fr.pose_map_src = up(side.data(), side.size());
+		LSFM_CHECK_HIP(hipStreamSynchronize(ctx->stream));
+		io.rhs = &fr;
+	}
 	h2d(ctx, io.x_pose, x_pose, (size_t)h.m * 6 * sizeof(double));
 	h2d(ctx, io.x_feat, x_feat, (size_t)h.n * 3 * sizeof(double));
 	int* d_small = ctx->scratch.alloc<int>(4);
```

Result: no change. 29.40 (median of 6 runs) (-0.6%).
